# paulvoliva/XNODE-WAN-PDE-solver

Measured on AMD Instinct MI355X. Metric: WAN training-steps/sec (optimiser sub-steps, d=20 cube, N_r=4096 paths per GPU), higher is better.
Workload: dtype f64

## Files before the change

### include/xnwan.h

```cpp
#ifndef XNWAN_H
#define XNWAN_H
#ifdef __cplusplus
extern "C" {
#endif

#define XW_E_DIMS     (-1)
#define XW_E_ARG      (-2)
#define XW_E_WORKSPACE (-3)
#define XW_E_COMM     (-4)

int xw_abi_version(void);
int xw_supported_dims(char* buf, int buflen);

int xw_theta_size(int d, int H, int K);
int xw_phi_size(int d, int W);

int xw_ode_fwd(const double* xT, const double* t, const double* start, const double* theta,
               int method, int N, int L, int d, int H, int K, int m,
               double* u, double* Y, void* stream);

typedef struct { const double* xT; const double* start; double* u; double* Y; double* act; int N;
                 int act_x_only;
                 int narrow;
                 int prio_drop;
               } XwOdeFwdJob;
int xw_ode_act_rows(int method, int H, int K, int m);
int xw_ode_fwd_multi(const XwOdeFwdJob* jobs, int njobs, const double* t, const double* theta,
                     int method, int L, int d, int H, int K, int m, double* zero16, void* stream);

int xw_ode_bwd_slabs(int N);

int xw_ode_bwd(const double* xT, const double* t, const double* start, const double* theta, const double* Y,
               const double* ubar, int method, int N, int L, int d, int H, int K, int m, int mode,
               double* gx, double* gs, double* gslab, void* stream);

typedef struct { const double* xT; const double* start; const double* Y; const double* act; const double* ubar;
                 double* gx; double* gs; double* gslab; int N;
                 int res_first_only; const double* res_u; const double* res_ref; double res_coef; double res_base;
                 int res_w_per_point; const double* res_w; const double* res_c; const double* res_cp; double res_kappa2;
               } XwOdeBwdJob;
int xw_ode_bwd_multi(const XwOdeBwdJob* jobs, int njobs, const double* t, const double* theta,
                     int method, int L, int d, int H, int K, int m, int mode, void* stream);

int xw_tiled_ode_ok(int d, int H, int K, int m);
int xw_tiled_ode_work(int sweep, int d, int H, int K, int m);
int xw_tiled_ode_bwd_slabs(int N);
int xw_tiled_ode_fwd_multi(const XwOdeFwdJob* jobs, int njobs, const double* t, const double* theta,
                           int method, int L, int d, int H, int K, int m, double* zero16, double* work, void* stream);
int xw_tiled_ode_bwd_multi(const XwOdeBwdJob* jobs, int njobs, const double* t, const double* theta,
                           int method, int L, int d, int H, int K, int m, int mode, double* work, void* stream);

int xw_adams_coef(int k, double* out);
int xw_adams_tiled_work(int sweep, int d, int H, int K, int m);
int xw_adams_tiled_fwd_multi(const XwOdeFwdJob* jobs, int njobs, const double* t, const double* theta,
                             int L, int d, int H, int K, int m, double* zero16, double* work, void* stream);
int xw_adams_tiled_bwd_multi(const XwOdeBwdJob* jobs, int njobs, const double* t, const double* theta,
                             int L, int d, int H, int K, int m, int mode, double* work, void* stream);

#define XW_DOPRI_CTL 16
#define XW_DOPRI_UNDERFLOW 1
#define XW_DOPRI_STEPS 2
#define XW_DOPRI_NONFINITE 3
#define XW_DOPRI_CAPACITY 4
typedef struct { const double* xT; const double* start; double* u; double* Y; double* rec_y; double* rec_t; double* rec_h;
                 double* fbuf; double* ctl; double* work; int N; int cap; } XwDopriJob;
int xw_dopri5_ctl_size(void);
int xw_dopri5_work_size(int N);
int xw_dopri5_init(const XwDopriJob* jobs, int njobs, const double* t, const double* theta, int L, int d, int H, int K, int m,
                   int Hn, double rtol, double atol, void* stream);
int xw_dopri5_attempts(const XwDopriJob* jobs, int njobs, const double* t, const double* theta, int L, int d, int H, int K,
                       int m, int Hn, double rtol, double atol, int max_steps, int n, void* stream);
typedef struct { XwOdeBwdJob b; const double* rec_y; const double* rec_t; const double* rec_h; const double* ctl; } XwDopriSweepJob;
int xw_dopri5_sweep(const XwDopriSweepJob* jobs, int njobs, const double* t, const double* theta, int L, int d, int H, int K,
                    int m, int mode, void* stream);

int xw_tdopri5_work(int sweep, int d, int H, int K, int m);
int xw_tdopri5_part_size(int N);
int xw_tdopri5_init(const XwDopriJob* jobs, int njobs, const double* t, const double* theta, int L, int d, int H, int K, int m,
                    int Hn, double rtol, double atol, double* work, void* stream);
int xw_tdopri5_attempts(const XwDopriJob* jobs, int njobs, const double* t, const double* theta, int L, int d, int H, int K,
                        int m, int Hn, double rtol, double atol, int max_steps, int n, double* work, void* stream);
int xw_tdopri5_sweep(const XwDopriSweepJob* jobs, int njobs, const double* t, const double* theta, int L, int d, int H, int K,
                     int m, int mode, double* work, void* stream);

int xw_disc_fwd(const double* xT, const double* t, const double* tpp, const double* phi,
                int N, int L, int d, int W, int q, double* v, double* vt, double* gxv, double* gtv, int ngrad,
                int max_blocks, double* act, void* stream);
int xw_disc_xproj(const double* xT, const double* phi, int N, int d, int W, double* xproj, void* stream);
int xw_disc_fwd_xproj(const double* xT, const double* t, const double* tpp, const double* phi,
                      int N, int L, int d, int W, int q, double* v, double* vt, double* gxv, double* gtv, int ngrad,
                      int max_blocks, double* act, const double* xproj, void* stream);
int xw_disc_act_rows(int W, int q);

int xw_disc_gradx(const double* xT, const double* t, const double* tpp, const double* phi, const double* vbar,
                  int N, int d, int W, int q, double* gxv, double* gtv, void* stream);

int xw_disc_bwd_slabs(int N, int L);
int xw_disc_bwd(const double* xT, const double* t, const double* tpp, const double* phi, const double* vbar,
                int N, int L, int d, int W, int q, const double* act, double* gslab, void* stream);

int xw_disc_tiled_ok(int d, int W, int q);
int xw_disc_tiled_act_rows(int W, int q);
int xw_disc_tiled_fwd(const double* xT, const double* t, const double* tpp, const double* phi,
                      int N, int L, int d, int W, int q, double* v, double* vt, double* gxv, double* gtv, int ngrad,
                      int max_blocks, double* act, const double* xproj, void* stream);
int xw_disc_tiled_bwd(const double* xT, const double* t, const double* tpp, const double* phi, const double* vbar,
                      int N, int L, int d, int W, int q, const double* act, double* gslab, void* stream);

int xw_weak_partials(const double* u, const double* v, const double* vt, const double* w, int w_per_point,
                     const double* wt, const double* s3x, const double* gx, const double* gs, const double* ghT,
                     const double* gxv, const double* w0, const double* gwx0T, int d, const double* c, double ckappa,
                     const double* f, const double* h, const double* href, int pairwise, double s3_scale, int N, int L,
                     double Vol, double Nglob, double* work, double* scal, int finalize, int Lb, double Nbglob, double alpha,
                     double init_off, double bdry_off, long long* step, const double* ub, const double* gb, long Pb,
                     void* stream);
int xw_pair_fold(double* scal, double Vol, double Nglob, void* stream);
int xw_reduce_work_size(void);
int xw_cube_weight(const float* x, int N, int d, double top, double bot, double* w, double* w0, double* gwT, double* xT,
                   void* stream);
int xw_weak_contract_general(const double* A0, int amode, const double* B0, const double* gx, const double* gs,
                             const double* ghT, const double* gxv, const double* w0, const double* gwx0T, const double* v0,
                             int d, int N, double* s3x, void* stream);
int xw_bdry_partials(const double* ub, const double* g, int Nb, int L, double alpha, double Nbglob,
                     double* ubar_b, double* work, double* scal, void* stream);
int xw_gen_cotangents(const double* u, const double* v, const double* w, int w_per_point, const double* c,
                      const double* cp, double ckappa, const double* h, int N, int L, double Vol, double Nglob,
                      double alpha, double pollution, const double* scal, double* ubarA, double* ubarB, void* stream);
int xw_disc_cotangent(const double* u, const double* v, const double* w, int w_per_point, const double* c,
                      double ckappa, const double* f, const double* h, int N, int L, double Vol, double Nglob,
                      double pollution, double s3_scale, const double* scal_in, double* vbar, void* stream);
int xw_losses(double* scal, int L, int Lb, double Vol, double Nglob, double Nbglob, double alpha, double init_off,
              double bdry_off, long long* step, void* stream);

int xw_adam(double* param, const double* gslabA, int nA, const double* gextraA, const double* gslabB, int nB,
            const double* gextraB, const double* scal, double* m, double* v, long long* step, int bump_step, int P,
            double lr, double beta1, double beta2, double eps, double* gsum_out, int lag_lo, int lag_hi, int skip,
            long long* lag, void* stream);
int xw_slab_sum(const double* gslab, int nslab, int P, int accumulate, double* out, void* stream);
int xw_slab_sum2(const double* gA, int nA, double* outA, const double* gB, int nB, double* outB, int P, void* stream);

typedef struct {
  int N, Nb, L, Lb, d;
  int same_grid;
  int w_per_point, amode, pair_i, pair_b;
  int ns_u, ns_b;
  int narrow;
  int sharded;
  double Vol, Nglob, Nbglob, s3_scale, init_off, bdry_off, ckappa;
  const double *xT, *xvT, *xbT, *t, *tb, *tpp, *xvT_pts;
  const double *start, *start_b, *h, *href, *f, *g, *w, *wt, *w0, *ghT, *gwx0T, *c, *cp, *A0, *B0;
  double *u, *ub, *Y, *Yb, *act, *act_b, *v, *vt, *gxv, *gtv, *gx, *gs, *vbar, *s3x, *vact, *slabA, *slabB, *slab_v, *work_i, *work_b;
  double *xproj;
} XwGroup;
typedef int (*XwExchangeFn)(double* buf, int count, void* ctx, void* stream);
typedef struct {
  int method, H, K, m, W, q, Pu, Pv, adjoint;
  int v_blocks, v_blocks_disc;
  int lag_lo, lag_hi;
  double alpha, pollution, lr_u, lr_v, beta1, beta2, eps;
  double *theta, *phi, *scal, *grad_u, *grad_v, *m_u, *v_u, *m_v, *v_v;
  long long *step_u, *step_v, *lag_u;
  XwExchangeFn exchange;
  void* exchange_ctx;
  double* pack_u;
} XwSolverState;
int xw_substep_gen(const XwGroup* g, const XwSolverState* s, int skip_v, int store_record, double* accum, int adam_skip_field,
                   void* stream);
int xw_substep_disc(const XwGroup* g, const XwSolverState* s, int skip_v, int use_record, double* accum, void* stream);

int xw_comm_available(void);
int xw_comm_unique_id(unsigned char* id128);
int xw_comm_init(const unsigned char* id128, int nranks, int rank, void** comm);
int xw_allreduce(double* buf, int count, void* comm, void* stream);
int xw_comm_destroy(void* comm);

typedef struct XwGather {
  const double* src;
  double* dst;
  long n0, n1, n2;
  long s0, s1, s2;
  long before;
} XwGather;
int xw_gather_fields(const XwGather* table_dev, int count, long total, void* stream);

int xw_mt19937_uniform_f32(void* state_blob, long blob_bytes, float* out, long n, float from, float to, int fused);

int xw_mt19937_legacy_normal_f64(unsigned int* key, int* pos, int* has_gauss, double* cached_gaussian, double* out, long n);

#ifdef __cplusplus
}
#endif
#endif
```

### xnode_wan_pde_solver_amd/_lib.py

```python
import ctypes
import os

_HERE = os.path.dirname(os.path.abspath(__file__))
LIB_PATH = os.environ.get('XW_LIBRARY') or os.path.join(_HERE, 'libxnwan.so')
ABI_VERSION = 33

c_f32p = ctypes.c_void_p
c_f64p = ctypes.c_void_p
c_i64p = ctypes.c_void_p
c_int, c_dbl, c_vp = ctypes.c_int, ctypes.c_double, ctypes.c_void_p


class XwOdeFwdJob(ctypes.Structure):
    _fields_ = [('xT', c_vp), ('start', c_vp), ('u', c_vp), ('Y', c_vp), ('act', c_vp), ('N', c_int), ('act_x_only', c_int),
                ('narrow', c_int), ('prio_drop', c_int)]


class XwOdeBwdJob(ctypes.Structure):
    _fields_ = [('xT', c_vp), ('start', c_vp), ('Y', c_vp), ('act', c_vp), ('ubar', c_vp), ('gx', c_vp), ('gs', c_vp),
                ('gslab', c_vp), ('N', c_int), ('res_first_only', c_int), ('res_u', c_vp), ('res_ref', c_vp),
                ('res_coef', ctypes.c_double), ('res_base', ctypes.c_double), ('res_w_per_point', c_int), ('res_w', c_vp),
                ('res_c', c_vp), ('res_cp', c_vp), ('res_kappa2', ctypes.c_double)]


class XwDopriJob(ctypes.Structure):
    _fields_ = [('xT', c_vp), ('start', c_vp), ('u', c_vp), ('Y', c_vp), ('rec_y', c_vp), ('rec_t', c_vp), ('rec_h', c_vp),
                ('fbuf', c_vp), ('ctl', c_vp), ('work', c_vp), ('N', c_int), ('cap', c_int)]


class XwDopriSweepJob(ctypes.Structure):
    _fields_ = [('b', XwOdeBwdJob), ('rec_y', c_vp), ('rec_t', c_vp), ('rec_h', c_vp), ('ctl', c_vp)]


class XwGroup(ctypes.Structure):
    _fields_ = ([(n, c_int) for n in ('N', 'Nb', 'L', 'Lb', 'd', 'same_grid', 'w_per_point', 'amode', 'pair_i', 'pair_b', 'ns_u', 'ns_b',
                                      'narrow', 'sharded')]
                + [(n, c_dbl) for n in ('Vol', 'Nglob', 'Nbglob', 's3_scale', 'init_off', 'bdry_off', 'ckappa')]
                + [(n, c_vp) for n in ('xT', 'xvT', 'xbT', 't', 'tb', 'tpp', 'xvT_pts', 'start', 'start_b', 'h', 'href', 'f', 'g', 'w',
                                       'wt', 'w0', 'ghT', 'gwx0T', 'c', 'cp', 'A0', 'B0', 'u', 'ub', 'Y', 'Yb', 'act', 'act_b', 'v',
                                       'vt', 'gxv', 'gtv', 'gx', 'gs', 'vbar', 's3x', 'vact', 'slabA', 'slabB', 'slab_v', 'work_i',
                                       'work_b', 'xproj')])


class XwSolverState(ctypes.Structure):
    _fields_ = ([(n, c_int) for n in ('method', 'H', 'K', 'm', 'W', 'q', 'Pu', 'Pv', 'adjoint', 'v_blocks', 'v_blocks_disc', 'lag_lo',
                                      'lag_hi')]
                + [(n, c_dbl) for n in ('alpha', 'pollution', 'lr_u', 'lr_v', 'beta1', 'beta2', 'eps')]
                + [(n, c_vp) for n in ('theta', 'phi', 'scal', 'grad_u', 'grad_v', 'm_u', 'v_u', 'm_v', 'v_v', 'step_u', 'step_v',
                                       'lag_u', 'exchange', 'exchange_ctx', 'pack_u')])


EXCHANGE_FN = ctypes.CFUNCTYPE(ctypes.c_int, ctypes.c_void_p, ctypes.c_int, ctypes.c_void_p, ctypes.c_void_p)


SIGNATURES = {
    'xw_abi_version': [],
    'xw_supported_dims': [ctypes.c_char_p, c_int],
    'xw_theta_size': [c_int, c_int, c_int],
    'xw_phi_size': [c_int, c_int],
    'xw_ode_fwd': [c_f32p, c_f32p, c_f64p, c_f64p, c_int, c_int, c_int, c_int, c_int, c_int, c_int, c_f64p, c_f64p, c_vp],
    'xw_ode_fwd_multi': [ctypes.POINTER(XwOdeFwdJob), c_int, c_f32p, c_f64p, c_int, c_int, c_int, c_int, c_int, c_int, c_f64p,
                         c_vp],
    'xw_ode_bwd_slabs': [c_int],
    'xw_ode_act_rows': [c_int, c_int, c_int, c_int],
    'xw_ode_bwd_multi': [ctypes.POINTER(XwOdeBwdJob), c_int, c_f32p, c_f64p, c_int, c_int, c_int, c_int, c_int, c_int, c_int, c_vp],
    'xw_tiled_ode_ok': [c_int, c_int, c_int, c_int],
    'xw_tiled_ode_work': [c_int, c_int, c_int, c_int, c_int],
    'xw_tiled_ode_bwd_slabs': [c_int],
    'xw_tiled_ode_fwd_multi': [ctypes.POINTER(XwOdeFwdJob), c_int, c_f32p, c_f64p, c_int, c_int, c_int, c_int, c_int, c_int, c_f64p,
                               c_f64p, c_vp],
    'xw_tiled_ode_bwd_multi': [ctypes.POINTER(XwOdeBwdJob), c_int, c_f32p, c_f64p, c_int, c_int, c_int, c_int, c_int, c_int, c_int,
                               c_f64p, c_vp],
    'xw_adams_coef': [c_int, c_vp],
    'xw_adams_tiled_work': [c_int, c_int, c_int, c_int, c_int],
    'xw_adams_tiled_fwd_multi': [ctypes.POINTER(XwOdeFwdJob), c_int, c_f32p, c_f64p, c_int, c_int, c_int, c_int, c_int, c_f64p, c_f64p,
                                 c_vp],
    'xw_adams_tiled_bwd_multi': [ctypes.POINTER(XwOdeBwdJob), c_int, c_f32p, c_f64p, c_int, c_int, c_int, c_int, c_int, c_int, c_f64p,
                                 c_vp],
    'xw_dopri5_ctl_size': [],
    'xw_dopri5_work_size': [c_int],
    'xw_dopri5_init': [ctypes.POINTER(XwDopriJob), c_int, c_f32p, c_f64p, c_int, c_int, c_int, c_int, c_int, c_int, c_dbl, c_dbl,
                       c_vp],
    'xw_dopri5_attempts': [ctypes.POINTER(XwDopriJob), c_int, c_f32p, c_f64p, c_int, c_int, c_int, c_int, c_int, c_int, c_dbl,
                           c_dbl, c_int, c_int, c_vp],
    'xw_dopri5_sweep': [ctypes.POINTER(XwDopriSweepJob), c_int, c_f32p, c_f64p, c_int, c_int, c_int, c_int, c_int, c_int, c_vp],
    'xw_tdopri5_work': [c_int, c_int, c_int, c_int, c_int],
    'xw_tdopri5_part_size': [c_int],
    'xw_tdopri5_init': [ctypes.POINTER(XwDopriJob), c_int, c_f32p, c_f64p, c_int, c_int, c_int, c_int, c_int, c_int, c_dbl, c_dbl,
                        c_f64p, c_vp],
    'xw_tdopri5_attempts': [ctypes.POINTER(XwDopriJob), c_int, c_f32p, c_f64p, c_int, c_int, c_int, c_int, c_int, c_int, c_dbl,
                            c_dbl, c_int, c_int, c_f64p, c_vp],
    'xw_tdopri5_sweep': [ctypes.POINTER(XwDopriSweepJob), c_int, c_f32p, c_f64p, c_int, c_int, c_int, c_int, c_int, c_int, c_f64p,
                         c_vp],
    'xw_ode_bwd': [c_f32p, c_f32p, c_f64p, c_f64p, c_f64p, c_f64p, c_int, c_int, c_int, c_int, c_int, c_int, c_int, c_int,
                   c_f64p, c_f64p, c_f64p, c_vp],
    'xw_disc_fwd': [c_f32p, c_f32p, c_f32p, c_f64p, c_int, c_int, c_int, c_int, c_int, c_f64p, c_f64p, c_f64p, c_f64p, c_int,
                    c_int, c_f64p, c_vp],
    'xw_disc_xproj': [c_f32p, c_f64p, c_int, c_int, c_int, c_f64p, c_vp],
    'xw_disc_fwd_xproj': [c_f32p, c_f32p, c_f32p, c_f64p, c_int, c_int, c_int, c_int, c_int, c_f64p, c_f64p, c_f64p, c_f64p, c_int,
                          c_int, c_f64p, c_f64p, c_vp],
    'xw_disc_act_rows': [c_int, c_int],
    'xw_disc_gradx': [c_f32p, c_f32p, c_f32p, c_f64p, c_f64p, c_int, c_int, c_int, c_int, c_f64p, c_f64p, c_vp],
    'xw_disc_bwd_slabs': [c_int, c_int],
    'xw_disc_bwd': [c_f32p, c_f32p, c_f32p, c_f64p, c_f64p, c_int, c_int, c_int, c_int, c_int, c_f64p, c_f64p, c_vp],
    'xw_disc_tiled_ok': [c_int, c_int, c_int],
    'xw_disc_tiled_act_rows': [c_int, c_int],
    'xw_disc_tiled_fwd': [c_f32p, c_f32p, c_f32p, c_f64p, c_int, c_int, c_int, c_int, c_int, c_f64p, c_f64p, c_f64p, c_f64p, c_int,
                          c_int, c_f64p, c_f64p, c_vp],
    'xw_disc_tiled_bwd': [c_f32p, c_f32p, c_f32p, c_f64p, c_f64p, c_int, c_int, c_int, c_int, c_int, c_f64p, c_f64p, c_vp],
    'xw_mt19937_uniform_f32': [c_vp, ctypes.c_long, c_vp, ctypes.c_long, ctypes.c_float, ctypes.c_float, c_int],
    'xw_gather_fields': [c_vp, c_int, ctypes.c_long, c_vp],
    'xw_mt19937_legacy_normal_f64': [c_vp, ctypes.POINTER(c_int), ctypes.POINTER(c_int), ctypes.POINTER(c_dbl), c_vp, ctypes.c_long],
    'xw_weak_partials': [c_f64p, c_f64p, c_f64p, c_f64p, c_int, c_f64p, c_f64p, c_f64p, c_f64p, c_f64p, c_f64p, c_f64p,
                         c_f64p, c_int, c_f64p, c_dbl, c_f64p, c_f64p, c_f64p, c_int, c_dbl, c_int, c_int, c_dbl, c_dbl, c_f64p, c_f64p,
                         c_int, c_int, c_dbl, c_dbl, c_dbl, c_dbl, c_i64p, c_f64p, c_f64p, ctypes.c_long, c_vp],
    'xw_pair_fold': [c_f64p, c_dbl, c_dbl, c_vp],
    'xw_cube_weight': [c_vp, c_int, c_int, c_dbl, c_dbl, c_f64p, c_f64p, c_f64p, c_f64p, c_vp],
    'xw_bdry_partials': [c_f64p, c_f64p, c_int, c_int, c_dbl, c_dbl, c_f64p, c_f64p, c_f64p, c_vp],
    'xw_reduce_work_size': [],
    'xw_weak_contract_general': [c_f64p, c_int, c_f64p, c_f64p, c_f64p, c_f64p, c_f64p, c_f64p, c_f64p, c_f64p, c_int, c_int, c_f64p, c_vp],
    'xw_gen_cotangents': [c_f64p, c_f64p, c_f64p, c_int, c_f64p, c_f64p, c_dbl, c_f64p, c_int, c_int, c_dbl, c_dbl, c_dbl,
                          c_dbl, c_f64p, c_f64p, c_f64p, c_vp],
    'xw_disc_cotangent': [c_f64p, c_f64p, c_f64p, c_int, c_f64p, c_dbl, c_f64p, c_f64p, c_int, c_int, c_dbl, c_dbl, c_dbl,
                          c_dbl, c_f64p, c_f64p, c_vp],
    'xw_losses': [c_f64p, c_int, c_int, c_dbl, c_dbl, c_dbl, c_dbl, c_dbl, c_dbl, c_i64p, c_vp],
    'xw_adam': [c_f64p, c_f64p, c_int, c_f64p, c_f64p, c_int, c_f64p, c_f64p, c_f64p, c_f64p, c_i64p, c_int, c_int, c_dbl,
                c_dbl, c_dbl, c_dbl, c_f64p, c_int, c_int, c_int, c_i64p, c_vp],
    'xw_substep_gen': [ctypes.POINTER(XwGroup), ctypes.POINTER(XwSolverState), c_int, c_int, c_f64p, c_int, c_vp],
    'xw_substep_disc': [ctypes.POINTER(XwGroup), ctypes.POINTER(XwSolverState), c_int, c_int, c_f64p, c_vp],
    'xw_slab_sum': [c_f64p, c_int, c_int, c_int, c_f64p, c_vp],
    'xw_slab_sum2': [c_f64p, c_int, c_f64p, c_f64p, c_int, c_f64p, c_int, c_vp],
    'xw_comm_available': [],
# ... 45 lines not shown
```

### xnode_wan_pde_solver_amd/csrc/xw_common.h

```cpp
#pragma once
#include <hip/hip_runtime.h>

typedef double d4 __attribute__((ext_vector_type(4)));
#define XW_MFMA(a, b, c) __builtin_amdgcn_mfma_f64_16x16x4f64((a), (b), (c), 0, 0, 0)
#define XW_MFMA4(a, b, c) __builtin_amdgcn_mfma_f64_4x4x4f64((a), (b), (c), 0, 0, 0)

#define XW_E_DIMS (-1)
#define XW_ODE_MAX_LAYERS 10
#define XW_E_ARG (-2)
#define XW_E_WORKSPACE (-3)
#define XW_E_COMM (-4)

struct UOff {
  int IL0w, IL0b, IL2w, IL2b, IL4w, IL4b, Win, Winb, Wh, Whb, Wo, Wob, FLw, FLb, total, ldin;
};
__host__ __device__ inline UOff u_offsets(int d, int H, int K) {
  UOff o;
  int p = 0;
  o.IL0w = p; p += H;
  o.IL0b = p; p += H;
  o.IL2w = p; p += H * H;
  o.IL2b = p; p += H;
  o.IL4w = p; p += H * H;
  o.IL4b = p; p += H;
  o.ldin = d + 1 + H;
  o.Win = p; p += K * o.ldin;
  o.Winb = p; p += K;
  o.Wh = p; p += K * K;
  o.Whb = p; p += K;
  o.Wo = p; p += H * K;
  o.Wob = p; p += H;
  o.FLw = p; p += H;
  o.FLb = p; p += 1;
  o.total = p;
  return o;
}
struct VOff {
  int Vin, Vinb, Vh, Vhb, Vo, Vob, total, ldin;
};
__host__ __device__ inline VOff v_offsets(int d, int W) {
  VOff o;
  int p = 0;
  o.ldin = d + 1;
  o.Vin = p; p += W * o.ldin;
  o.Vinb = p; p += W;
  o.Vh = p; p += W * W;
  o.Vhb = p; p += W;
  o.Vo = p; p += W;
  o.Vob = p; p += 1;
  o.total = p;
  return o;
}

typedef const double __attribute__((address_space(1)))* xw_gcp;
typedef double __attribute__((address_space(1)))* xw_gp;
__device__ __forceinline__ double xw_ld_g(const double* p) { return *(xw_gcp)p; }
__device__ __forceinline__ void xw_st_g(double v, double* p) { *(xw_gp)p = v; }
__device__ __forceinline__ double xw_ld_nt(const double* p) { return __builtin_nontemporal_load((xw_gcp)p); }
__device__ __forceinline__ void xw_st_nt(double v, double* p) { __builtin_nontemporal_store(v, (xw_gp)p); }

__device__ __forceinline__ int xw_lane() { return threadIdx.x & 63; }

__device__ __forceinline__ double xw_fragA(const double* __restrict__ Mx, int ld, int rows, int cols, int r0, int c0) {
  const int l = xw_lane();
  const int r = r0 + (l & 15), c = c0 + (l >> 4);
  return (r < rows && c < cols) ? xw_ld_g(Mx + (r * ld + c)) : 0.0;
}
__device__ __forceinline__ double xw_fragAT(const double* __restrict__ Mx, int ld, int rows, int cols, int r0, int c0) {
  const int l = xw_lane();
  const int r = r0 + (l & 15), c = c0 + (l >> 4);
  return (r < cols && c < rows) ? xw_ld_g(Mx + (c * ld + r)) : 0.0;
}
__device__ __forceinline__ double xw_fragAT_l(const double* __restrict__ Mx, int ld, int rows, int cols, int r0, int c0, int l) {
  const int r = r0 + (l & 15), c = c0 + (l >> 4);
  return (r < cols && c < rows) ? xw_ld_g(Mx + (c * ld + r)) : 0.0;
}
__device__ __forceinline__ double xw_fragA4(const double* __restrict__ Mx, int ld, int rows, int cols, int r0, int c0) {
  const int l = xw_lane();
  const int r = r0 + (l & 3), c = c0 + (l >> 4);
  return (r < rows && c < cols) ? xw_ld_g(Mx + (r * ld + c)) : 0.0;
}
__device__ __forceinline__ double xw_fragAT4(const double* __restrict__ Mx, int ld, int rows, int cols, int r0, int c0) {
  const int l = xw_lane();
  const int r = r0 + (l & 3), c = c0 + (l >> 4);
  return (r < cols && c < rows) ? xw_ld_g(Mx + (c * ld + r)) : 0.0;
}
__device__ __forceinline__ double xw_relu1(double x) { return __builtin_fmax(x, 0.0); }
__device__ __forceinline__ d4 xw_vecD(const double* __restrict__ b, int rows, int r0) {
  const int g = xw_lane() >> 4;
  d4 v;
#pragma unroll
  for (int r = 0; r < 4; ++r) {
    const int i = r0 + g + 4 * r;
    v[r] = (i < rows) ? xw_ld_g(b + i) : 0.0;
  }
  return v;
}
__device__ __forceinline__ d4 xw_vecD_strided(const double* __restrict__ b, int stride, int rows, int r0) {
  const int g = xw_lane() >> 4;
  d4 v;
#pragma unroll
  for (int r = 0; r < 4; ++r) {
    const int i = r0 + g + 4 * r;
    v[r] = (i < rows) ? xw_ld_g(b + (long)i * stride) : 0.0;
  }
  return v;
}
__device__ __forceinline__ d4 xw_relu(d4 z) {
  d4 o;
#pragma unroll
  for (int r = 0; r < 4; ++r) o[r] = z[r] > 0.0 ? z[r] : 0.0;
  return o;
}
__device__ __forceinline__ double xw_gate_pos(double b, double x) {
  const unsigned t = (unsigned)__double2loint(b) | (unsigned)__double2hiint(b);
  const int m = -(int)(t < 1u ? t : 1u);
  return __hiloint2double(__double2hiint(x) & m, __double2loint(x) & m);
}
__device__ __forceinline__ d4 xw_zero4() { d4 z = {0.0, 0.0, 0.0, 0.0}; return z; }

__device__ __forceinline__ double xw_tanh(double x) {
  const double am = fmin(fabs(x), 40.0);
  const double y = -2.0 * am;
  const double nb = fma(y, 1.4426950408889634, 6755399441055744.0);
  const double n = nb - 6755399441055744.0;
  double r = fma(n, -6.93147180369123816490e-01, y);
  r = fma(n, -1.90821492927058770002e-10, r);
  double p = 2.08767569878681e-09;
  p = fma(p, r, 2.505210838544172e-08);
  p = fma(p, r, 2.755731922398589e-07);
  p = fma(p, r, 2.7557319223985893e-06);
  p = fma(p, r, 2.48015873015873e-05);
  p = fma(p, r, 0.0001984126984126984);
  p = fma(p, r, 0.001388888888888889);
  p = fma(p, r, 0.008333333333333333);
  p = fma(p, r, 0.041666666666666664);
  p = fma(p, r, 0.16666666666666666);
  p = fma(p, r, 0.5);
  p = fma(p, r, 1.0);
  p = fma(p, r, 1.0);
  const double e = __hiloint2double(__double2hiint(p) + (__double2loint(nb) << 20), __double2loint(p));
  const double num = 1.0 - e, den = 1.0 + e;
// ... 74 lines not shown
```

### xnode_wan_pde_solver_amd/csrc/xw_dopri.hip

```cpp
#include "xw_common.h"
#include "xnwan.h"
#include "xw_generic.h"

namespace {
#include "xw_generic_field.h"
#include "xw_generic_cot.h"

#include "xw_dopri_ctl.h"

__device__ __forceinline__ void put_output(const XwDopriJob& j, const double* flw, double flb, int l, int H, int path,
                                           const double* y) {
  double acc = flb;
  for (int h = 0; h < H; ++h) acc = fma(flw[h], y[h], acc);
  j.u[(long)l * j.N + path] = acc;
  if (j.Y)
    for (int h = 0; h < H; ++h) j.Y[((long)l * H + h) * j.N + path] = y[h];
}

template <int HM>
__global__ void __launch_bounds__(64) kd_init1(const Jobs<XwDopriJob> J, const double* __restrict__ tf, const double* __restrict__ theta,
                                               int L, int d, int H, int K, int m, int Hn, double rtol, double atol) {
  int lb;
  const XwDopriJob& j = J.j[job_of(J, lb)];
  const int N = j.N, nb = (N + 63) / 64, raw = lb * 64 + (int)threadIdx.x;
// ... 302 lines not shown
  const double* Win = theta + n.o.Win;
  if (slab) {
    gadd_run(slab, n.o.Winb, K, active, [&](int q) { return Sx[q]; });
    for (int q = 0; q < K; ++q) {
      const double sq = Sx[q];
      gadd_run(slab, n.o.Win + q * n.o.ldin, d, active, [&](int i) { return sq * job.xT[(long)i * N + path]; });
    }
  }
  if (want_x && job.gx != nullptr && active)
    for (int i = 0; i < d; ++i) {
      double acc = 0.0;
      for (int q = 0; q < K; ++q) acc = fma(Win[q * n.o.ldin + i], Sx[q], acc);
      job.gx[(long)i * N + path] = acc;
    }
}

bool dims_ok(int L, int d, int H, int K, int m, int Hn) { return L >= 1 && xwg_ode_ok(d, H, K, m) && Hn >= 1 && Hn <= H; }

int fwd_jobs(const XwDopriJob* jobs, int njobs, Jobs<XwDopriJob>& P) {
  int e = pack_jobs(jobs, njobs, P);
  if (e) return e;
  for (int i = 0; i < njobs; ++i) {
    const XwDopriJob& j = jobs[i];
    if (!j.xT || !j.start || !j.u || !j.rec_y || !j.rec_t || !j.rec_h || !j.fbuf || !j.ctl || !j.work || j.N < 1 || j.cap < 0)
      return XW_E_ARG;
    P.blk0[i + 1] = P.blk0[i] + (j.N + 63) / 64;
  }
  return 0;
}
}

extern "C" int xw_dopri5_ctl_size(void) { return XW_DOPRI_CTL; }
extern "C" int xw_dopri5_work_size(int N) { return N < 1 ? XW_E_ARG : 2 * ((N + 63) / 64); }

extern "C" int xw_dopri5_init(const XwDopriJob* jobs, int njobs, const double* t, const double* theta, int L, int d, int H, int K,
                              int m, int Hn, double rtol, double atol, void* stream) {
  if (!t || !theta || !(rtol >= 0.0) || !(atol >= 0.0)) return XW_E_ARG;
  if (!dims_ok(L, d, H, K, m, Hn)) return XW_E_DIMS;
  Jobs<XwDopriJob> P;
  const int e = fwd_jobs(jobs, njobs, P);
  if (e) return e;
  hipStream_t s = (hipStream_t)stream;
  const dim3 g(P.blk0[njobs]), b(64);
  if (H <= 32) {
    hipLaunchKernelGGL(kd_init1<32>, g, b, 0, s, P, t, theta, L, d, H, K, m, Hn, rtol, atol);
    hipLaunchKernelGGL(kd_init2<32>, g, b, 0, s, P, t, theta, L, d, H, K, m, Hn, rtol, atol);
  } else {
    hipLaunchKernelGGL(kd_init1<64>, g, b, 0, s, P, t, theta, L, d, H, K, m, Hn, rtol, atol);
    hipLaunchKernelGGL(kd_init2<64>, g, b, 0, s, P, t, theta, L, d, H, K, m, Hn, rtol, atol);
  }
  return xw_launch_status();
}

extern "C" int xw_dopri5_attempts(const XwDopriJob* jobs, int njobs, const double* t, const double* theta, int L, int d, int H,
                                  int K, int m, int Hn, double rtol, double atol, int max_steps, int n, void* stream) {
  if (!t || !theta || !(rtol >= 0.0) || !(atol >= 0.0) || max_steps < 1 || n < 0) return XW_E_ARG;
  if (!dims_ok(L, d, H, K, m, Hn)) return XW_E_DIMS;
  Jobs<XwDopriJob> P;
  const int e = fwd_jobs(jobs, njobs, P);
  if (e) return e;
  hipStream_t s = (hipStream_t)stream;
  const dim3 g(P.blk0[njobs]), b(64);
  for (int i = 0; i < n; ++i) {
    if (H <= 32)
      hipLaunchKernelGGL(kd_attempt<32>, g, b, 0, s, P, t, theta, L, d, H, K, m, Hn, rtol, atol, max_steps);
    else
      hipLaunchKernelGGL(kd_attempt<64>, g, b, 0, s, P, t, theta, L, d, H, K, m, Hn, rtol, atol, max_steps);
  }
  return xw_launch_status();
}

extern "C" int xw_dopri5_sweep(const XwDopriSweepJob* jobs, int njobs, const double* t, const double* theta, int L, int d, int H,
                               int K, int m, int mode, void* stream) {
  if (!t || !theta || L < 1 || (mode & ~7) || ((mode & 4) && (mode & 3) != 3)) return XW_E_ARG;
  if (!xwg_ode_ok(d, H, K, m)) return XW_E_DIMS;
  Jobs<XwDopriSweepJob> P;
  int e = pack_jobs(jobs, njobs, P);
  if (e) return e;
  hipStream_t s = (hipStream_t)stream;
  const long Pu = u_offsets(d, H, K).total;
  for (int i = 0; i < njobs; ++i) {
    const XwDopriSweepJob& j = jobs[i];
    if (!j.b.xT || !j.b.start || !j.rec_y || !j.rec_t || !j.rec_h || !j.ctl || j.b.N < 1) return XW_E_ARG;
    if (j.b.res_u != nullptr && j.b.ubar != nullptr) return XW_E_ARG;
    if ((mode & 2) && !j.b.gslab) return XW_E_ARG;
    if ((mode & 1) && !(mode & 4) && (!j.b.gx || !j.b.gs)) return XW_E_ARG;
    if (mode & 2) {
      const hipError_t he = hipMemsetAsync(j.b.gslab, 0, sizeof(double) * Pu * ((j.b.N + 15) / 16), s);
      if (he != hipSuccess) return (int)he;
    }
    P.blk0[i + 1] = P.blk0[i] + (j.b.N + 63) / 64;
  }
  const dim3 g(P.blk0[njobs]), b(64);
  if (H <= 32)
    hipLaunchKernelGGL(kd_sweep<32>, g, b, 0, s, P, t, theta, L, d, H, K, m, mode);
  else
    hipLaunchKernelGGL(kd_sweep<64>, g, b, 0, s, P, t, theta, L, d, H, K, m, mode);
  return xw_launch_status();
}
```

### xnode_wan_pde_solver_amd/csrc/xw_generic.hip

```cpp
#include "xw_common.h"
#include "xnwan.h"
#include "xw_generic.h"

namespace {
#include "xw_generic_field.h"

__device__ void rk_step(const Net& n, int method, const double* xproj, double t0, double dt, double* y) {
  const int H = n.H;
  double k1[GH], k2[GH], k3[GH], tmp[GH];
  field_eval(n, xproj, t0, y, k1, nullptr);
  if (method == 0) {
    for (int j = 0; j < H; ++j) y[j] = fma(dt, k1[j], y[j]);
  } else if (method == 1) {
    for (int j = 0; j < H; ++j) tmp[j] = fma(k1[j], dt / 2, y[j]);
    field_eval(n, xproj, t0 + dt / 2, tmp, k2, nullptr);
    for (int j = 0; j < H; ++j) y[j] = fma(dt, k2[j], y[j]);
  } else {
    for (int j = 0; j < H; ++j) tmp[j] = y[j] + dt * k1[j] / 3;
    field_eval(n, xproj, t0 + dt / 3, tmp, k2, nullptr);
    for (int j = 0; j < H; ++j) tmp[j] = y[j] + dt * (k2[j] - k1[j] / 3);
    field_eval(n, xproj, t0 + 2 * dt / 3, tmp, k3, nullptr);
    for (int j = 0; j < H; ++j) tmp[j] = y[j] + dt * (k1[j] - k2[j] + k3[j]);
    double k4[GH];
    field_eval(n, xproj, t0 + dt, tmp, k4, nullptr);
// ... 294 lines not shown
        dj[kk] = r[(long)kk * cols] > 0.0 ? a0 : 0.0;
        if (kk + 1 < W) dj[kk + 1] = r[(long)(kk + 1) * cols] > 0.0 ? a1 : 0.0;
        if (kk + 2 < W) dj[kk + 2] = r[(long)(kk + 2) * cols] > 0.0 ? a2 : 0.0;
        if (kk + 3 < W) dj[kk + 3] = r[(long)(kk + 3) * cols] > 0.0 ? a3 : 0.0;
      }
    }
    for (int k = 0; k < W; k += 4) {
      double dk[4][GQ];
#pragma unroll
      for (int j = 0; j < GQ; ++j)
#pragma unroll
        for (int i = 0; i < 4; ++i) dk[i][j] = (j < q && k + i < W) ? dls[(j + 1) * GW + k + i] : 0.0;
      const int lane = threadIdx.x;
      for (int c = 0; c < W; c += 64) {
        double mine[4] = {0.0, 0.0, 0.0, 0.0};
        for (int i = 0; i < 64; ++i) {
          if (c + i >= W) break;
          double a0 = 0.0, a1 = 0.0, a2 = 0.0, a3 = 0.0;
#pragma unroll
          for (int j = 0; j < GQ; ++j) {
            if (j < q) {
              const double rj = act[((long)j * W + c + i) * cols + p];
              a0 = fma(dk[0][j], rj, a0);
              a1 = fma(dk[1][j], rj, a1);
              a2 = fma(dk[2][j], rj, a2);
              a3 = fma(dk[3][j], rj, a3);
            }
          }
          a0 = gsum64(a0); a1 = gsum64(a1); a2 = gsum64(a2); a3 = gsum64(a3);
          if (lane == i) { mine[0] = a0; mine[1] = a1; mine[2] = a2; mine[3] = a3; }
        }
        if (c + lane < W) {
#pragma unroll
          for (int i = 0; i < 4; ++i)
            if (k + i < W) slab[o.Vh + (k + i) * W + c + lane] += mine[i];
        }
      }
    }
    wadd_run(slab, o.Vhb, W, [&](int k) {
      double acc = 0.0;
      for (int j = 0; j < q; ++j) acc += dls[(j + 1) * GW + k];
      return acc;
    });
    wadd_run(slab, o.Vinb, W, [&](int k) { return dls[k]; });
    for (int k = 0; k < W; ++k) {
      const double d0 = dls[k];
      wadd_run(slab, o.Vin + k * o.ldin, 1 + d, [&](int c) { return d0 * (c == 0 ? t : xT[(long)(c - 1) * N + nidx]); });
    }
  }
}

}

int xwg_ode_ok(int d, int H, int K, int m) { return H >= 1 && H <= GH && K >= 1 && K <= GK && m >= 1 && m <= GM && d >= 1 && d + 2 <= 128; }
int xwg_disc_ok(int d, int W, int q) { return W >= 1 && W <= GW && q >= 0 && q <= GQ && d >= 1 && d + 2 <= 128; }

int xwg_ode_fwd_multi(const XwOdeFwdJob* jobs, int njobs, const double* t, const double* theta, int method, int L, int d, int H,
                      int K, int m, double* zero16, void* stream) {
  if (!jobs || njobs < 1 || !t || !theta || L < 1 || method < 0 || method > 2) return XW_E_ARG;
  if (!xwg_ode_ok(d, H, K, m)) return XW_E_DIMS;
  hipStream_t s = (hipStream_t)stream;
  if (zero16 != nullptr) {
    const hipError_t e = hipMemsetAsync(zero16, 0, 16 * sizeof(double), s);
    if (e != hipSuccess) return (int)e;
  }
  for (int i = 0; i < njobs; ++i) {
    const XwOdeFwdJob& j = jobs[i];
    if (!j.xT || !j.start || !j.u || j.N < 1) return XW_E_ARG;
    hipLaunchKernelGGL(kg_ode_fwd, dim3((j.N + 63) / 64), dim3(64), 0, s, j, t, theta, method, L, d, H, K, m);
  }
  return xw_launch_status();
}

int xwg_ode_bwd_multi(const XwOdeBwdJob* jobs, int njobs, const double* t, const double* theta, int method, int L, int d, int H,
                      int K, int m, int mode, void* stream) {
  if (!jobs || njobs < 1 || !t || !theta || L < 1 || method < 0 || method > 2 || (mode & 3) == 0) return XW_E_ARG;
  if (!xwg_ode_ok(d, H, K, m) || (mode & 8)) return XW_E_DIMS;
  if ((mode & 4) && (mode & 3) != 3) return XW_E_ARG;
  hipStream_t s = (hipStream_t)stream;
  const long P = u_offsets(d, H, K).total;
  for (int i = 0; i < njobs; ++i) {
    const XwOdeBwdJob& j = jobs[i];
    if (!j.xT || !j.start || !j.Y || j.N < 1) return XW_E_ARG;
    if (j.res_u != nullptr && j.ubar != nullptr) return XW_E_ARG;
    if ((mode & 2) && !j.gslab) return XW_E_ARG;
    if ((mode & 1) && !(mode & 4) && (!j.gx || !j.gs)) return XW_E_ARG;
    if (mode & 2) {
      const hipError_t e = hipMemsetAsync(j.gslab, 0, sizeof(double) * P * ((j.N + 15) / 16), s);
      if (e != hipSuccess) return (int)e;
    }
    hipLaunchKernelGGL(kg_ode_bwd, dim3((j.N + 63) / 64), dim3(64), 0, s, j, t, theta, method, L, d, H, K, m, mode);
  }
  return xw_launch_status();
}

int xwg_disc_fwd(const double* xT, const double* t, const double* tpp, const double* phi, int N, int L, int d, int W, int q,
                 double* v, double* vt, double* gxv, double* gtv, int ngrad, double* act, void* stream) {
  if (!xwg_disc_ok(d, W, q)) return XW_E_DIMS;
  const long P = (long)N * L;
  const long cols = (P + 15) / 16 * 16;
  hipLaunchKernelGGL(kg_disc_fwd, dim3((unsigned)((P + 63) / 64)), dim3(64), 0, (hipStream_t)stream, xT, t, tpp, phi, N, L, d, W, q, v,
                     vt, gxv, gtv, ngrad, act, cols);
  return xw_launch_status();
}

int xwg_disc_bwd(const double* xT, const double* t, const double* tpp, const double* phi, const double* vbar, int N, int L, int d,
                 int W, int q, const double* act, double* gslab, int nslab, void* stream) {
  if (!xwg_disc_ok(d, W, q)) return XW_E_DIMS;
  if (!act) return XW_E_DIMS;
  const long P = (long)N * L;
  const long cols = (P + 15) / 16 * 16;
  const hipError_t e = hipMemsetAsync(gslab, 0, sizeof(double) * (size_t)v_offsets(d, W).total * nslab, (hipStream_t)stream);
  if (e != hipSuccess) return (int)e;
  hipLaunchKernelGGL(kg_disc_bwd, dim3(nslab), dim3(64), 0, (hipStream_t)stream, xT, t, tpp, phi, vbar, N, L, d, W, q, act, cols, gslab);
  return xw_launch_status();
}
```

### xnode_wan_pde_solver_amd/csrc/xw_generic_cot.h

```cpp
#pragma once
__device__ double cot_u(const XwOdeBwdJob& j, int l, int L, int path) {
  const long p = (long)l * j.N + path;
  if (j.res_u == nullptr) return j.ubar ? j.ubar[p] : 1.0;
  if (j.res_first_only == 2) {
    const double u = j.res_u[p], v = j.res_ref[p];
    const double w = j.res_w_per_point ? j.res_w[p] : j.res_w[path];
    const double dcu = j.res_c != nullptr ? j.res_c[p] + u * j.res_cp[p] : j.res_kappa2 * u;
    double g = j.res_coef * dcu * v * w;
    if (l == L - 1) g += j.res_base * v;
    return g;
  }
  if (j.res_first_only == 1) return l == 0 ? j.res_base + j.res_coef * (j.res_u[p] - j.res_ref[path]) : j.res_base;
  return j.res_base + j.res_coef * (j.res_u[p] - j.res_ref[p]);
}
```

### xnode_wan_pde_solver_amd/csrc/xw_ode.hip

```cpp
#include <cstdlib>
#include <type_traits>
#include "xw_common.h"
#ifndef XW_ODE_FWD_WAVES
#define XW_ODE_FWD_WAVES 2
#endif
#include "xnwan.h"

#if !defined(XW_ODE_H) || !defined(XW_ODE_K)
#error "compile with -DXW_ODE_H=<u_hidden_dim> -DXW_ODE_K=<u_hidden_hidden_dim>"
#endif
#ifdef XW_ODE_WIDE16
#define XW_ODE_FORM "xw_ode_mfma16.h"
#else
#define XW_ODE_FORM "xw_ode_mfma4.h"
#endif
#define XW_CAT4_(a, b, c, d) a##b##c##d
#define XW_CAT4(a, b, c, d) XW_CAT4_(a, b, c, d)
#define XW_ODE_FN(name) XW_CAT4(name, XW_ODE_H, _, XW_ODE_K)
#ifdef XW_ODE_ONLY_M
#define XW_ODE_DISPATCH(CALL)                                    \
  switch (m) {                                                   \
    case XW_ODE_ONLY_M: { CALL(XW_ODE_H, XW_ODE_K, XW_ODE_ONLY_M) } \
    default: return XW_E_DIMS;                                   \
  }
// ... 179 lines not shown
#pragma unroll
  for (int ks = 0; ks < 4; ++ks) acc = XW_MFMA(a[ks], b[ks], acc);
  __builtin_amdgcn_sched_barrier(0);
}
#define XW_SWEEP_TILES 6

#define XW_ODE_SECTION 1
#include XW_ODE_FORM
template <int H, int K>
__device__ __forceinline__ void lift(const double* __restrict__ th, const UOff& o, double sv, d4 (&a0)[Dim<H, K>::HT],
                                     d4 (&a1)[Dim<H, K>::HT], d4 (&y)[Dim<H, K>::HT]) {
  typedef Dim<H, K> D;
#pragma unroll
  for (int ht = 0; ht < D::HT; ++ht)
    a0[ht] = xw_relu(xw_vecD(th + o.IL0w, H, 16 * ht) * sv + xw_vecD(th + o.IL0b, H, 16 * ht));
#pragma unroll
  for (int ht = 0; ht < D::HT; ++ht) {
    d4 v = xw_vecD(th + o.IL2b, H, 16 * ht);
#pragma unroll
    for (int ks = 0; ks < D::KSH; ++ks) v = XW_MFMA(xw_fragA(th + o.IL2w, H, H, H, 16 * ht, 4 * ks), a0[ks >> 2][ks & 3], v);
    a1[ht] = xw_relu(v);
  }
#pragma unroll
  for (int ht = 0; ht < D::HT; ++ht) {
    d4 v = xw_vecD(th + o.IL4b, H, 16 * ht);
#pragma unroll
    for (int ks = 0; ks < D::KSH; ++ks) v = XW_MFMA(xw_fragA(th + o.IL4w, H, H, H, 16 * ht, 4 * ks), a1[ks >> 2][ks & 3], v);
    y[ht] = v;
  }
}

template <int H, int K>
__device__ __forceinline__ d4 project_x(const double* __restrict__ th, const UOff& o, const double* __restrict__ xT,
                                        int N, int d, int ncl) {
  const int g = xw_lane() >> 4;
  d4 xp = xw_vecD(th + o.Winb, K, 0);
  for (int ks = 0; ks < (d + 3) / 4; ++ks) {
    const int i = 4 * ks + g;
    const double b = i < d ? xT[(long)i * N + ncl] : 0.0;
    xp = XW_MFMA(xw_fragA(th + o.Win, o.ldin, K, d, 0, 4 * ks), b, xp);
  }
  return xp;
}

#define XW_MAXJOBS 4
struct FwdJobs {
  const double* xT[XW_MAXJOBS];
  const double* start[XW_MAXJOBS];
  double* u[XW_MAXJOBS];
  double* Y[XW_MAXJOBS];
  double* act[XW_MAXJOBS];
  int N[XW_MAXJOBS];
  int tile0[XW_MAXJOBS + 1];
  int n;
  int x_only;
  int narrow;
  int prio;
  double* zero16;
};
struct BwdJobs {
  const double* xT[XW_MAXJOBS];
  const double* start[XW_MAXJOBS];
  const double* Y[XW_MAXJOBS];
  const double* act[XW_MAXJOBS];
  const double* ubar[XW_MAXJOBS];
  double* gx[XW_MAXJOBS];
  double* gs[XW_MAXJOBS];
  double* gslab[XW_MAXJOBS];
  int N[XW_MAXJOBS];
  int tile0[XW_MAXJOBS + 1];
  int n;
  int x_ones;
  int prio;
  int spread;
  const double* res_u[XW_MAXJOBS];
  const double* res_ref[XW_MAXJOBS];
  double res_coef[XW_MAXJOBS], res_base[XW_MAXJOBS];
  int res_first[XW_MAXJOBS];
  const double* res_w[XW_MAXJOBS];
  const double* res_c[XW_MAXJOBS];
  const double* res_cp[XW_MAXJOBS];
  double res_kappa2[XW_MAXJOBS];
  int res_wpp[XW_MAXJOBS];
};
__device__ __forceinline__ double cot_u(const BwdJobs& jobs, int job, const double* __restrict__ ubar, int l, int N, int col,
                                        int L) {
  const double* __restrict__ ru = jobs.res_u[job];
  if (ru != nullptr) {
    if (jobs.res_first[job] == 2) {
      const long p = (long)l * N + col;
      const double ul = ru[p], vl = jobs.res_ref[job][p];
      const double wl = jobs.res_wpp[job] ? jobs.res_w[job][p] : jobs.res_w[job][col];
      const double dcu = jobs.res_c[job] != nullptr ? jobs.res_c[job][p] + ul * jobs.res_cp[job][p] : jobs.res_kappa2[job] * ul;
      double gB = jobs.res_coef[job] * dcu * vl * wl;
      if (l == L - 1) gB += jobs.res_base[job] * vl;
      return gB;
    }
    double r = jobs.res_base[job];
    if (jobs.res_first[job]) {
      if (l == 0) r += jobs.res_coef[job] * (ru[col] - jobs.res_ref[job][col]);
    } else {
      r += jobs.res_coef[job] * (ru[(long)l * N + col] - jobs.res_ref[job][(long)l * N + col]);
    }
    return r;
  }
  return ubar != nullptr ? ubar[(long)l * N + col] : 1.0;
}
struct Cot4 {
  const double *p0, *p1, *p2, *p3, *p4;
  long s0, s1, s2;
  double cb, coef, base, kappa2;
  bool weak, use_st, use_res, first, tab, valid;
};
struct CotRaw { double a, b, c, d, e; };
__device__ __forceinline__ Cot4 make_cot(const BwdJobs& jobs, int job, int N, int col, bool valid, const double* dummy) {
  Cot4 c;
  const double* ru = jobs.res_u[job];
  const double* ubar = jobs.ubar[job];
  c.valid = valid;
  c.weak = ru != nullptr && jobs.res_first[job] == 2;
  c.use_res = ru != nullptr && !c.weak;
  c.use_st = ru == nullptr && ubar != nullptr;
  c.first = c.use_res && jobs.res_first[job] != 0;
  c.cb = ru != nullptr ? jobs.res_base[job] : (ubar != nullptr ? 0.0 : 1.0);
  c.coef = jobs.res_coef[job];
  c.base = jobs.res_base[job];
  c.kappa2 = jobs.res_kappa2[job];
  c.tab = c.weak && jobs.res_c[job] != nullptr;
  if (c.weak) {
    c.p0 = ru + col; c.p1 = jobs.res_ref[job] + col; c.p2 = jobs.res_w[job] + col;
    c.p3 = (c.tab ? jobs.res_c[job] : ru) + col; c.p4 = (c.tab ? jobs.res_cp[job] : ru) + col;
    c.s0 = N; c.s1 = N; c.s2 = jobs.res_wpp[job] ? N : 0;
  } else {
    c.p0 = (c.use_st ? ubar : dummy) + col; c.s0 = c.use_st ? N : 0;
    c.p1 = (c.use_res ? ru : dummy) + col; c.p2 = (c.use_res ? jobs.res_ref[job] : dummy) + col;
    c.s1 = (c.use_res && !c.first) ? N : 0; c.s2 = 0;
    c.p3 = c.p4 = dummy;
  }
  return c;
}
template <bool WEAK> __device__ __forceinline__ CotRaw cot_issue(const Cot4& c, int l) {
  CotRaw r;
  r.a = xw_ld_g(c.p0 + l * c.s0);
  r.b = xw_ld_g(c.p1 + l * c.s1);
  if (WEAK) {
    r.c = xw_ld_g(c.p2 + l * c.s2);
    r.d = xw_ld_g(c.p3 + l * c.s1);
    r.e = xw_ld_g(c.p4 + l * c.s1);
  } else {
    r.c = xw_ld_g(c.p2 + l * c.s1);
    r.d = r.e = 0.0;
  }
  return r;
}
template <bool WEAK> __device__ __forceinline__ double cot_value(const Cot4& c, const CotRaw& r, int l, int L) {
  double ub;
  if (WEAK) {
    const double dcu = c.tab ? fma(r.a, r.e, r.d) : c.kappa2 * r.a;
    ub = c.coef * dcu * r.b * r.c;
    if (l == L - 1) ub = fma(c.base, r.b, ub);
  } else {
    ub = c.cb;
    if (c.use_st) ub += r.a;
    if (c.use_res && (!c.first || l == 0)) ub = fma(c.coef, r.b - r.c, ub);
  }
  return c.valid ? ub : 0.0;
}

template <typename J> __device__ __forceinline__ int find_job(const J& jobs, int vb) {
  int j = 0;
#pragma unroll
  for (int k = 1; k < XW_MAXJOBS; ++k)
    if (k < jobs.n && vb >= jobs.tile0[k]) j = k;
  return j;
}

#define XW_ODE_PRIO 3
__device__ __forceinline__ void xw_setprio(int p) {
  if (p >= 3) __builtin_amdgcn_s_setprio(3);
  else if (p == 2) __builtin_amdgcn_s_setprio(2);
  else if (p == 1) __builtin_amdgcn_s_setprio(1);
}

template <int H, int K, int M, int S> struct ActLayout {
  static constexpr int STAGE = M * K;
  static constexpr int YI = S * STAGE;
  static constexpr int ROWS = S * STAGE + (S - 1) * H;
  static constexpr int MASK = ROWS;
  static constexpr int MR = 2 * XW_MASK_WORDS(M);
  static constexpr int TOTAL = ROWS + MR * S;
};
struct ActLane {
  unsigned off;
  unsigned off_part;
  unsigned off_part_st;
  bool valid;
};
#define XW_ACT_OOB 0x7fffff00u
__device__ __forceinline__ ActLane act_lane(int N, int col, bool valid, int krows) {
  const int g = xw_lane() >> 4, p = krows & 3;
  const int gp = p ? (g < p ? g : p - 1) : g;
  const unsigned part = 8u * (unsigned)((p ? p : 4) * col + gp);
  return ActLane{8u * (unsigned)(4 * col + g), part, (p == 0 || g < p) ? part : XW_ACT_OOB, valid};
}
typedef unsigned xw_u2v __attribute__((ext_vector_type(2)));
struct ActBuf {
  __amdgpu_buffer_rsrc_t rsrc;
};
__device__ __forceinline__ ActBuf act_buf(double* A, int bytes) {
  return ActBuf{__builtin_amdgcn_make_buffer_rsrc(A, 0, bytes, 0x00020000)};
}
__device__ __forceinline__ void act_store(const ActBuf& B, int row0, int nrows, int N, const ActLane& q, d4 v) {
#pragma unroll
  for (int r = 0; r < 4; ++r)
    if (4 * r < nrows) {
      const int so = (row0 + 4 * r) * N * 8;
      const double x = v[r];
      const xw_u2v w2 = {(unsigned)__double2loint(x), (unsigned)__double2hiint(x)};
      __builtin_amdgcn_raw_buffer_store_b64(w2, B.rsrc, (int)(4 * r + 4 <= nrows ? q.off : q.off_part_st), so, 2);
    }
}
__device__ __forceinline__ d4 act_load(const double* __restrict__ A, int row0, int nrows, int N, const ActLane& q) {
  d4 v = xw_zero4();
  const char* base = reinterpret_cast<const char*>(A + (long)row0 * N);
#pragma unroll
  for (int r = 0; r < 4; ++r)
    if (4 * r < nrows) {
      const char* __restrict__ blk = base + (long)(4 * r) * N * 8;
      v[r] = __builtin_nontemporal_load(reinterpret_cast<const double*>(blk + (4 * r + 4 <= nrows ? q.off : q.off_part)));
    }
  return v;
}

template <int K, int M, bool FULL = true> struct SinkAct {
  const ActBuf& A;
  int row0, N;
  const ActLane& q;
  unsigned& bits;
  unsigned& bits_hi;
  __device__ __forceinline__ double relu(int, int kb, double z) const {
    const bool kb_last = kb == (K + 3) / 4 - 1;
    const unsigned long long open = __builtin_amdgcn_ballot_w64(z > 0.0);
    double r;
    if constexpr (XW_MASK_WORDS(M) == 2) {
      if (kb_last) asm("v_addc_co_u32_e64 %1, vcc, %1, %1, %4\n\tv_addc_co_u32_e64 %2, vcc, %2, %2, vcc\n\tv_max_f64 %0, %3, 0\n\ts_nop 1" : "=v"(r), "+v"(bits), "+v"(bits_hi) : "v"(z), "s"(open) : "vcc");
      else asm("v_addc_co_u32_e64 %1, vcc, %1, %1, %4\n\tv_addc_co_u32_e64 %2, vcc, %2, %2, vcc\n\tv_max_f64 %0, %3, 0" : "=v"(r), "+v"(bits), "+v"(bits_hi) : "v"(z), "s"(open) : "vcc");
      return r;
// ... 682 lines not shown
  for (int i = 0; i < jobs.n; ++i) act = act && jobs.act[i] != nullptr;
  const int sel = method * 3 + (act ? (jobs.x_only ? 2 : 1) : 0);
  int rc;
  if (launch_fwd_narrow<H, K, M>(sel, jobs, t, theta, L, d, grid, s, rc)) return rc;
  switch (sel) {
    case 0: hipLaunchKernelGGL((k_ode_fwd<H, K, M, 0, 0>), grid, block, 0, s, jobs, t, theta, L, d); break;
    case 1: hipLaunchKernelGGL((k_ode_fwd<H, K, M, 0, 1>), grid, block, 0, s, jobs, t, theta, L, d); break;
    case 2: hipLaunchKernelGGL((k_ode_fwd<H, K, M, 0, 2>), grid, block, 0, s, jobs, t, theta, L, d); break;
    case 3: hipLaunchKernelGGL((k_ode_fwd<H, K, M, 1, 0>), grid, block, 0, s, jobs, t, theta, L, d); break;
    case 4: hipLaunchKernelGGL((k_ode_fwd<H, K, M, 1, 1>), grid, block, 0, s, jobs, t, theta, L, d); break;
    case 5: hipLaunchKernelGGL((k_ode_fwd<H, K, M, 1, 2>), grid, block, 0, s, jobs, t, theta, L, d); break;
    case 6: hipLaunchKernelGGL((k_ode_fwd<H, K, M, 2, 0>), grid, block, 0, s, jobs, t, theta, L, d); break;
    default: return XW_E_ARG;
  }
  return xw_launch_status();
}

}

#ifndef XW_ODE_PART_RECOMP
extern "C" int XW_ODE_FN(xw_ode_fwd_multi_w)(const XwOdeFwdJob* jobs, int njobs, const double* t, const double* theta, int method,
                                             int L, int d, int m, double* zero16, void* stream) {
  if (!jobs || njobs < 1 || njobs > XW_MAXJOBS || !t || !theta || L <= 0 || d <= 0 || m < 1) return XW_E_ARG;
  FwdJobs J;
  J.n = njobs;
  J.zero16 = zero16;
  J.x_only = jobs[0].act_x_only ? 1 : 0;
  J.narrow = jobs[0].narrow ? 1 : 0;
  J.prio = XW_ODE_PRIO - (jobs[0].prio_drop < 0 ? 0 : jobs[0].prio_drop > 3 ? 3 : jobs[0].prio_drop);
  J.tile0[0] = 0;
  for (int i = 0; i < XW_MAXJOBS; ++i) {
    const bool on = i < njobs;
    if (on && (!jobs[i].xT || !jobs[i].start || !jobs[i].u || jobs[i].N <= 0)) return XW_E_ARG;
    if (on && (jobs[i].act_x_only ? 1 : 0) != J.x_only) return XW_E_ARG;
    if (on && (jobs[i].narrow ? 1 : 0) != J.narrow) return XW_E_ARG;
    J.xT[i] = on ? jobs[i].xT : nullptr;
    J.start[i] = on ? jobs[i].start : nullptr;
    J.u[i] = on ? jobs[i].u : nullptr;
    J.Y[i] = on ? jobs[i].Y : nullptr;
    J.act[i] = (on && method != 2) ? jobs[i].act : nullptr;
    if (on && (J.act[i] != nullptr) != (J.act[0] != nullptr)) return XW_E_ARG;
    J.N[i] = on ? jobs[i].N : 0;
    J.tile0[i + 1] = J.tile0[i] + (on ? (jobs[i].N + 15) / 16 : 0);
  }
  hipStream_t s = (hipStream_t)stream;
#define CALL(HH, KK, MM) return launch_fwd<HH, KK, MM>(method, J, t, theta, L, d, s);
  XW_ODE_DISPATCH(CALL)
#undef CALL
}

extern "C" int XW_ODE_FN(xw_ode_bwd_multi_w)(const XwOdeBwdJob* jobs, int njobs, const double* t, const double* theta, int method,
                                             int L, int d, int m, int mode, void* stream) {
  if (!jobs || njobs < 1 || njobs > XW_MAXJOBS || !t || !theta || L <= 0 || d <= 0 || m < 1 || (mode & 3) == 0 || ((mode & 4) && (mode & 3) != 3) || ((mode & 8) && (mode & 4)) || ((mode & 16) && (mode & 8)) || (mode & ~127)) return XW_E_ARG;
  BwdJobs J;
  J.n = njobs;
  J.x_ones = (mode & 4) ? 1 : 0;
  J.spread = 0;
  J.prio = XW_ODE_PRIO - ((mode >> 5) & 3);
  J.tile0[0] = 0;
  for (int i = 0; i < XW_MAXJOBS; ++i) {
    const bool on = i < njobs;
    if (on) {
      if (!jobs[i].xT || !jobs[i].start || !jobs[i].Y || jobs[i].N <= 0) return XW_E_ARG;
      if ((mode & 2) && !jobs[i].gslab) return XW_E_ARG;
      if ((mode & 1) && !(mode & 4) && (!jobs[i].gx || !jobs[i].gs)) return XW_E_ARG;
      if ((mode & 1) && (!jobs[i].gx != !jobs[i].gs)) return XW_E_ARG;
    }
    J.xT[i] = on ? jobs[i].xT : nullptr;
    J.start[i] = on ? jobs[i].start : nullptr;
    J.Y[i] = on ? jobs[i].Y : nullptr;
    J.act[i] = (on && method != 2 && !(mode & 8)) ? jobs[i].act : nullptr;
    if (on && (J.act[i] != nullptr) != (J.act[0] != nullptr)) return XW_E_ARG;
    J.ubar[i] = on ? jobs[i].ubar : nullptr;
    J.res_u[i] = on ? jobs[i].res_u : nullptr;
    J.res_ref[i] = on ? jobs[i].res_ref : nullptr;
    J.res_coef[i] = on ? jobs[i].res_coef : 0.0;
    J.res_base[i] = on ? jobs[i].res_base : 0.0;
    J.res_first[i] = on ? jobs[i].res_first_only : 0;
    J.res_w[i] = on ? jobs[i].res_w : nullptr;
    J.res_c[i] = on ? jobs[i].res_c : nullptr;
    J.res_cp[i] = on ? jobs[i].res_cp : nullptr;
    J.res_kappa2[i] = on ? jobs[i].res_kappa2 : 0.0;
    J.res_wpp[i] = on ? jobs[i].res_w_per_point : 0;
    if (on && jobs[i].res_u && (!jobs[i].res_ref || jobs[i].ubar)) return XW_E_ARG;
    if (on && jobs[i].res_u && jobs[i].res_first_only == 2 && (!jobs[i].res_w || (!jobs[i].res_c != !jobs[i].res_cp))) return XW_E_ARG;
    if (on && (jobs[i].res_first_only < 0 || jobs[i].res_first_only > 2)) return XW_E_ARG;
    J.gx[i] = (on && (mode & 1)) ? jobs[i].gx : nullptr;
    J.gs[i] = (on && (mode & 1)) ? jobs[i].gs : nullptr;
    J.gslab[i] = (on && (mode & 2)) ? jobs[i].gslab : nullptr;
    J.N[i] = on ? jobs[i].N : 0;
    J.tile0[i + 1] = J.tile0[i] + (on ? (jobs[i].N + 15) / 16 : 0);
  }
  hipStream_t s = (hipStream_t)stream;
#define CALL(HH, KK, MM)                                                             \
  return (mode & 2) ? launch_bwd<HH, KK, MM, true>(method, J, t, theta, L, d, (mode & 8) != 0, (mode & 16) != 0, s)     \
                    : launch_bwd<HH, KK, MM, false>(method, J, t, theta, L, d, (mode & 8) != 0, (mode & 16) != 0, s);
  XW_ODE_DISPATCH(CALL)
#undef CALL
}
#else
extern "C" int XW_ODE_FN(xw_ode_bwd_recomp_w)(const void* jobs_, const double* t, const double* theta, int method, int L, int d,
                                              int m, int params, int adj, void* stream) {
  const BwdJobs& jobs = *static_cast<const BwdJobs*>(jobs_);
  const dim3 grid(jobs.tile0[jobs.n]), block(64);
  hipStream_t s = (hipStream_t)stream;
#define LAUNCH(HH, KK, MM, PP, AA)                                                                                                 \
  switch (method) {                                                                                                                \
    case 0: hipLaunchKernelGGL((k_ode_bwd<HH, KK, MM, 0, PP, false, AA>), grid, block, 0, s, jobs, t, theta, L, d); break;         \
    case 1: hipLaunchKernelGGL((k_ode_bwd<HH, KK, MM, 1, PP, false, AA>), grid, block, 0, s, jobs, t, theta, L, d); break;         \
    case 2: hipLaunchKernelGGL((k_ode_bwd<HH, KK, MM, 2, PP, false, AA>), grid, block, 0, s, jobs, t, theta, L, d); break;         \
    default: return XW_E_ARG;                                                                                                      \
  }                                                                                                                                \
  return xw_launch_status();
#define CALL(HH, KK, MM)                                                                                                           \
  if (params && adj) { LAUNCH(HH, KK, MM, true, true) }                                                                            \
  else if (params) { LAUNCH(HH, KK, MM, true, false) }                                                                             \
  else if (adj) { LAUNCH(HH, KK, MM, false, true) }                                                                                \
  else { LAUNCH(HH, KK, MM, false, false) }
  XW_ODE_DISPATCH(CALL)
#undef CALL
#undef LAUNCH
}
#endif
```

### xnode_wan_pde_solver_amd/csrc/xw_substep.hip

```cpp
#include <hip/hip_runtime.h>
#include <string.h>
#include "xnwan.h"

namespace {
struct Side {
  hipStream_t s = nullptr;
  hipEvent_t fork = nullptr, fwd = nullptr, done = nullptr;
};
Side* side_of_current_device() {
  static Side sides[64];
  int dev = 0;
  if (hipGetDevice(&dev) != hipSuccess || dev < 0 || dev >= 64) return nullptr;
  Side& x = sides[dev];
  if (x.s == nullptr) {
    if (hipStreamCreateWithFlags(&x.s, hipStreamNonBlocking) != hipSuccess) return nullptr;
    if (hipEventCreateWithFlags(&x.fork, hipEventDisableTiming) != hipSuccess || hipEventCreateWithFlags(&x.fwd, hipEventDisableTiming) != hipSuccess ||
        hipEventCreateWithFlags(&x.done, hipEventDisableTiming) != hipSuccess)
      return nullptr;
  }
  return &x;
}
#define XW_HIP(call) { const hipError_t e_ = (call); if (e_ != hipSuccess) return (int)e_; }

inline XwOdeFwdJob fwd_job(const double* xT, const double* start, double* u, double* Y, double* act, int N, int x_only, int narrow) {
  XwOdeFwdJob j;
  j.xT = xT; j.start = start; j.u = u; j.Y = Y; j.act = act; j.N = N; j.act_x_only = x_only; j.narrow = narrow; j.prio_drop = 0;
  return j;
}
inline XwOdeBwdJob bwd_job(const double* xT, const double* start, const double* Y, const double* act, int N) {
  XwOdeBwdJob j;
  memset(&j, 0, sizeof(j));
  j.xT = xT; j.start = start; j.Y = Y; j.act = act; j.N = N;
  return j;
}
#define XW_TRY(call) { const int rc_ = (call); if (rc_ != 0) return rc_; }

int test_net(const XwGroup* g, const XwSolverState* s, int blocks, double* record, void* stream) {
  if (g->tpp != nullptr)
    return xw_disc_fwd(g->xvT_pts, nullptr, g->tpp, s->phi, g->N * g->L, 1, g->d, s->W, s->q, g->v, g->vt, g->gxv, g->gtv, g->N, blocks,
                       record, stream);
  if (g->xproj != nullptr) XW_TRY(xw_disc_xproj(g->xvT, s->phi, g->N, g->d, s->W, g->xproj, stream));
  return xw_disc_fwd_xproj(g->xvT, g->t, nullptr, s->phi, g->N, g->L, g->d, s->W, s->q, g->v, g->vt, g->gxv, g->gtv, g->N, blocks, record,
                           g->xproj, stream);
}
int contract(const XwGroup* g, const XwSolverState* s, long long* step, bool with_bdry, bool finalize, void* stream) {
  const double* s3x = nullptr;
  if (g->A0 != nullptr || g->B0 != nullptr) {
    XW_TRY(xw_weak_contract_general(g->A0, g->amode, g->B0, g->gx, g->gs, g->ghT, g->gxv, g->w0, g->gwx0T, g->v, g->d, g->N, g->s3x,
                                    stream));
    s3x = g->s3x;
  }
  const bool fused = s3x == nullptr;
  return xw_weak_partials(g->u, g->v, g->vt, g->w, g->w_per_point, g->wt, s3x, fused ? g->gx : nullptr, fused ? g->gs : nullptr,
                          fused ? g->ghT : nullptr, fused ? g->gxv : nullptr, fused ? g->w0 : nullptr, fused ? g->gwx0T : nullptr,
                          fused ? g->d : 0, g->c, g->ckappa, g->f, g->h, g->pair_i ? g->href : nullptr, g->pair_i ? 1 : 0,
                          g->pair_i ? g->s3_scale : 1.0, g->N, g->L, g->Vol, g->Nglob, g->work_i, s->scal, finalize ? 1 : 0,
                          g->Lb > 0 ? g->Lb : 1, g->Nbglob, s->alpha, g->init_off, g->bdry_off, finalize ? step : nullptr, with_bdry && g->Nb > 0 ? g->ub : nullptr,
                          with_bdry && g->Nb > 0 ? g->g : nullptr, with_bdry && g->Nb > 0 ? (long)g->Nb * g->Lb : 0, stream);
}
inline bool sharded(const XwGroup* g, const XwSolverState* s) { return g->sharded != 0 && s->exchange != nullptr; }
#define XW_ZERO(ptr, count) XW_HIP(hipMemsetAsync((ptr), 0, sizeof(double) * (size_t)(count), (hipStream_t)stream))
}

extern "C" int xw_substep_gen(const XwGroup* g, const XwSolverState* s, int skip_v, int store_record, double* accum,
                              int adam_skip_field, void* stream) {
  if (!g || !s || g->N < 0 || g->Nb < 0 || g->L <= 0) return XW_E_ARG;
  const bool shard = sharded(g, s);
  if (g->N == 0 && !shard) return XW_E_ARG;
  if (shard && (!s->pack_u || s->scal != s->pack_u + 2 * (long)s->Pu)) return XW_E_ARG;
  const bool fused_x = s->pollution == 1.0 && !s->adjoint;
  const bool have_i = g->N > 0, have_b = g->Nb > 0;
  const bool joint = have_i && have_b && g->same_grid;
  const int adj = s->adjoint ? 8 : 0;
  void* const main_stream = stream;
  if (have_i) {
    Side* sd = side_of_current_device();
    if (sd == nullptr) return XW_E_ARG;
    XW_HIP(hipEventRecord(sd->fork, (hipStream_t)main_stream));
    XW_HIP(hipStreamWaitEvent(sd->s, sd->fork, 0));
    if (!skip_v) XW_TRY(test_net(g, s, s->v_blocks, store_record ? g->vact : nullptr, main_stream));
    stream = (void*)sd->s;
    {
      XwOdeFwdJob jobs[2] = {fwd_job(g->xT, g->start, g->u, g->Y, g->act, g->N, 0, (g->narrow >> 0) & 1),
                             fwd_job(g->xbT, g->start_b, g->ub, g->Yb, g->act_b, g->Nb, 0, (g->narrow >> 0) & 1)};
      XW_TRY(xw_ode_fwd_multi(jobs, joint ? 2 : 1, g->t, s->theta, s->method, g->L, g->d, s->H, s->K, s->m, s->scal, stream));
      if (have_b && !joint) {
        XwOdeFwdJob jb = fwd_job(g->xbT, g->start_b, g->ub, g->Yb, g->act_b, g->Nb, 0, (g->narrow >> 1) & 1);
        XW_TRY(xw_ode_fwd_multi(&jb, 1, g->tb, s->theta, s->method, g->Lb, g->d, s->H, s->K, s->m, nullptr, stream));
      }
    }
    XW_HIP(hipEventRecord(sd->fwd, sd->s));
    stream = main_stream;
    XW_HIP(hipStreamWaitEvent((hipStream_t)main_stream, sd->fwd, 0));
  } else {
    XW_ZERO(s->scal, 16);
    if (have_b) {
      XwOdeFwdJob jb = fwd_job(g->xbT, g->start_b, g->ub, g->Yb, g->act_b, g->Nb, 0, (g->narrow >> 1) & 1);
      XW_TRY(xw_ode_fwd_multi(&jb, 1, g->tb, s->theta, s->method, g->Lb, g->d, s->H, s->K, s->m, nullptr, stream));
    }
  }
  if (have_i && !fused_x) {
    XwOdeBwdJob jx = bwd_job(g->xT, g->start, g->Y, g->act, g->N);
    jx.gx = g->gx; jx.gs = g->gs;
    XW_TRY(xw_ode_bwd_multi(&jx, 1, g->t, s->theta, s->method, g->L, g->d, s->H, s->K, s->m, 1 | adj | (((g->narrow >> 5) & 1) ? 16 : 0),
                            stream));
  }
  {
    XwOdeBwdJob jobs[3];
    int nj = 0;
    if (have_i) {
      jobs[nj] = bwd_job(g->xT, g->start, g->Y, g->act, g->N);
      jobs[nj].gslab = g->slabA;
      if (fused_x) { jobs[nj].gx = g->gx; jobs[nj].gs = g->gs; }
      jobs[nj].res_u = g->u; jobs[nj].res_ref = g->pair_i ? g->href : g->h; jobs[nj].res_first_only = 1;
      jobs[nj].res_coef = 2.0 * s->alpha / g->Nglob; jobs[nj].res_base = s->pollution;
      ++nj;
    }
    XwOdeBwdJob jb = bwd_job(g->xbT, g->start_b, g->Yb, g->act_b, g->Nb);
    if (have_b) {
      jb.gslab = g->slabA + (long)g->ns_u * s->Pu;
      jb.res_u = g->ub; jb.res_ref = g->g; jb.res_first_only = 0;
      jb.res_coef = 2.0 * s->alpha / (g->Nbglob * g->Lb); jb.res_base = 0.0;
    }
    if (joint) jobs[nj++] = jb;
    if (have_i) {
      XwOdeBwdJob jB = bwd_job(g->xT, g->start, g->Y, g->act, g->N);
      jB.gslab = g->slabB;
      jB.res_first_only = 2; jB.res_u = g->u; jB.res_ref = g->v;
      jB.res_coef = g->Vol / g->Nglob / g->L * g->s3_scale; jB.res_base = g->Vol / g->Nglob;
      jB.res_w_per_point = g->w_per_point; jB.res_w = g->w; jB.res_c = g->c; jB.res_cp = g->cp; jB.res_kappa2 = 2.0 * g->ckappa;
      jobs[nj++] = jB;
      const int modeA = (fused_x ? (1 | 2 | 4) : 2) | adj | (((g->narrow >> 2) & 1) ? 16 : 0);
      XW_TRY(xw_ode_bwd_multi(jobs, nj, g->t, s->theta, s->method, g->L, g->d, s->H, s->K, s->m, modeA, stream));
    }
    if (have_b && !joint)
      XW_TRY(xw_ode_bwd_multi(&jb, 1, g->tb, s->theta, s->method, g->Lb, g->d, s->H, s->K, s->m, 2 | adj | (((g->narrow >> 3) & 1) ? 16 : 0),
                              stream));
  }
  if (have_i) {
    XW_TRY(contract(g, s, s->step_u, true, !shard, stream));
  } else if (have_b) {
    XW_TRY(xw_bdry_partials(g->ub, g->g, g->Nb, g->Lb, s->alpha, g->Nbglob, nullptr, g->work_b, s->scal, stream));
  }
  if (!shard) {
    XW_TRY(xw_adam(s->theta, g->slabA, g->ns_u + g->ns_b, accum, g->slabB, g->ns_u, nullptr, s->scal, s->m_u, s->v_u, s->step_u, -1, s->Pu,
                   s->lr_u, s->beta1, s->beta2, s->eps, s->grad_u, s->lag_lo, s->lag_hi, adam_skip_field, s->lag_u, stream));
  } else {
    const int nA = (have_i ? g->ns_u : 0) + (have_b ? g->ns_b : 0), nB = have_i ? g->ns_u : 0;
    double* const pA = s->pack_u;
    double* const pB = s->pack_u + s->Pu;
    if (nA > 0 && nB > 0) {
      XW_TRY(xw_slab_sum2(g->slabA, nA, pA, g->slabB, nB, pB, s->Pu, stream));
    } else {
      if (nA > 0) { XW_TRY(xw_slab_sum(g->slabA + (have_i ? 0 : (long)g->ns_u * s->Pu), nA, s->Pu, 0, pA, stream)); } else { XW_ZERO(pA, s->Pu); }
      XW_ZERO(pB, s->Pu);
    }
    XW_TRY(s->exchange(s->pack_u, 2 * s->Pu + 16, s->exchange_ctx, stream));
// ... 73 lines not shown
```

### xnode_wan_pde_solver_amd/csrc/xw_tdopri.hip

```cpp
#include "xw_common.h"
#include "xnwan.h"

namespace {
#include "xw_tiled_blocks.h"
#include "xw_generic_cot.h"

__device__ __forceinline__ double gsum64(double x) { return xw_sum_over_g(xw_sum_over_n(x)); }

#include "xw_dopri_ctl.h"

struct TdWork {
  TileWork w;
  long k, total;
};
__host__ __device__ inline TdWork td_work(int sweep, int d, int H, int K, int m) {
  TdWork q;
  q.w = tile_work(sweep, d, H, K, m);
  q.k = q.w.total;
  q.total = q.w.total + 16L * H * (sweep ? 14 : 7);
  return q;
}

__device__ __forceinline__ void tload(int H, int N, int p0, const double* __restrict__ src, double* v) {
  for (int e = lane_id(); e < 16 * H; e += 64) {
// ... 344 lines not shown
    touter(slab, n.o.Win, n.o.ldin, K, d, Sx, ws + w.xt, A_PLAIN);
  }
  if (want_x && job.gx != nullptr) {
    double* gxt = ws + w.xt + 16L * d;
    tgemm(theta + n.o.Win, 1, n.o.ldin, d, K, Sx, A_PLAIN, nullptr, nullptr, 0, 0.0, nullptr, E_NONE, nullptr, gxt);
    for (int e = lane_id(); e < 16 * d; e += 64)
      if (p0 + (e & 15) < N) job.gx[(long)(e >> 4) * N + p0 + (e & 15)] = gxt[e];
  }
}

bool dims_ok(int d, int H, int K, int m) { return xw_tiled_ode_ok(d, H, K, m) != 0; }

int fwd_check(int njobs, const double* t, const double* theta, int L, int d, int H, int K, int m, int Hn, double rtol, double atol,
              const double* work) {
  if (!t || !theta || !work || L < 1 || njobs < 1 || njobs > XW_DOPRI_MAXJOBS || !(rtol >= 0.0) || !(atol >= 0.0)) return XW_E_ARG;
  if (!dims_ok(d, H, K, m)) return XW_E_DIMS;
  if (Hn < 1 || Hn > H) return XW_E_ARG;
  return 0;
}

int fwd_jobs(const XwDopriJob* jobs, int njobs, Jobs<XwDopriJob>& P) {
  const int e = pack_jobs(jobs, njobs, P);
  if (e) return e;
  for (int i = 0; i < njobs; ++i) {
    const XwDopriJob& j = jobs[i];
    if (!j.xT || !j.start || !j.u || !j.rec_y || !j.rec_t || !j.rec_h || !j.fbuf || !j.ctl || !j.work || j.N < 1 || j.cap < 0)
      return XW_E_ARG;
    P.blk0[i + 1] = P.blk0[i] + (j.N + 15) / 16;
  }
  return 0;
}
}

extern "C" int xw_tdopri5_work(int sweep, int d, int H, int K, int m) {
  if (!dims_ok(d, H, K, m)) return XW_E_DIMS;
  return (int)td_work(sweep != 0, d, H, K, m).total;
}

extern "C" int xw_tdopri5_part_size(int N) { return N < 1 ? XW_E_ARG : 2 * ((N + 15) / 16); }

extern "C" int xw_tdopri5_init(const XwDopriJob* jobs, int njobs, const double* t, const double* theta, int L, int d, int H, int K,
                               int m, int Hn, double rtol, double atol, double* work, void* stream) {
  int e = fwd_check(njobs, t, theta, L, d, H, K, m, Hn, rtol, atol, work);
  if (e) return e;
  Jobs<XwDopriJob> P;
  e = fwd_jobs(jobs, njobs, P);
  if (e) return e;
  hipStream_t s = (hipStream_t)stream;
  const dim3 g(P.blk0[njobs]), b(64);
  hipLaunchKernelGGL(kq_init1, g, b, 0, s, P, t, theta, L, d, H, K, m, Hn, rtol, atol, work);
  hipLaunchKernelGGL(kq_init2, g, b, 0, s, P, t, theta, L, d, H, K, m, Hn, rtol, atol, work);
  return xw_launch_status();
}

extern "C" int xw_tdopri5_attempts(const XwDopriJob* jobs, int njobs, const double* t, const double* theta, int L, int d, int H,
                                   int K, int m, int Hn, double rtol, double atol, int max_steps, int n, double* work,
                                   void* stream) {
  int e = fwd_check(njobs, t, theta, L, d, H, K, m, Hn, rtol, atol, work);
  if (e) return e;
  if (max_steps < 1 || n < 0) return XW_E_ARG;
  Jobs<XwDopriJob> P;
  e = fwd_jobs(jobs, njobs, P);
  if (e) return e;
  hipStream_t s = (hipStream_t)stream;
  const dim3 g(P.blk0[njobs]), b(64);
  for (int i = 0; i < n; ++i)
    hipLaunchKernelGGL(kq_attempt, g, b, 0, s, P, t, theta, L, d, H, K, m, Hn, rtol, atol, max_steps, work);
  return xw_launch_status();
}

extern "C" int xw_tdopri5_sweep(const XwDopriSweepJob* jobs, int njobs, const double* t, const double* theta, int L, int d, int H,
                                int K, int m, int mode, double* work, void* stream) {
  if (!t || !theta || !work || L < 1 || njobs < 1 || njobs > XW_DOPRI_MAXJOBS) return XW_E_ARG;
  if ((mode & 3) == 0 || (mode & ~31) || ((mode & 4) && (mode & 3) != 3)) return XW_E_ARG;
  if (!dims_ok(d, H, K, m) || (mode & (8 | 16))) return XW_E_DIMS;
  Jobs<XwDopriSweepJob> P;
  const int e = pack_jobs(jobs, njobs, P);
  if (e) return e;
  hipStream_t s = (hipStream_t)stream;
  const long Pu = u_offsets(d, H, K).total;
  for (int i = 0; i < njobs; ++i) {
    const XwDopriSweepJob& j = jobs[i];
    if (!j.b.xT || !j.b.start || !j.rec_y || !j.rec_t || !j.rec_h || !j.ctl || j.b.N < 1) return XW_E_ARG;
    if (j.b.res_u != nullptr && j.b.ubar != nullptr) return XW_E_ARG;
    if ((mode & 2) && !j.b.gslab) return XW_E_ARG;
    if ((mode & 1) && !(mode & 4) && (!j.b.gx || !j.b.gs)) return XW_E_ARG;
    P.blk0[i + 1] = P.blk0[i] + (j.b.N + 15) / 16;
  }
  if (mode & 2)
    for (int i = 0; i < njobs; ++i) {
      const hipError_t he = hipMemsetAsync(jobs[i].b.gslab, 0, sizeof(double) * Pu * ((jobs[i].b.N + 15) / 16), s);
      if (he != hipSuccess) return (int)he;
    }
  hipLaunchKernelGGL(kq_sweep, dim3(P.blk0[njobs]), dim3(64), 0, s, P, t, theta, L, d, H, K, m, mode, work);
  return xw_launch_status();
}
```

### xnode_wan_pde_solver_amd/csrc/xw_tiled.hip

```cpp
#include "xw_common.h"
#include "xnwan.h"

namespace {
#include "xw_tiled_blocks.h"

#define XWA_HIST 11

struct AbRows { double b[XWA_HIST + 1][XWA_HIST]; };
__host__ __device__ constexpr AbRows ab_rows() {
  AbRows r{};
  for (int k = 1; k <= XWA_HIST; ++k)
    for (int j = 0; j < k; ++j) {
      long long c[XWA_HIST + 1] = {1};
      int deg = 0;
      for (int i = 0; i < k; ++i) {
        if (i == j) continue;
        for (int p = deg + 1; p >= 1; --p) c[p] = c[p - 1] + (long long)i * c[p];
        c[0] *= i;
        ++deg;
      }
      long long num = 0, den = 27720;
      for (int p = 0; p <= deg; ++p) num += c[p] * (27720 / (p + 1));
      for (int i = 2; i <= j; ++i) den *= i;
      for (int i = 2; i <= k - 1 - j; ++i) den *= i;
// ... 383 lines not shown
      touter(slab, n.o.IL2w, H, H, H, dh2, p0v, A_RELU);
      trowsum(slab, n.o.IL4b, 1, H, l0, nullptr, 1.0);
      trowsum(slab, n.o.IL2b, 1, H, dh2, nullptr, 1.0);
      trowsum(slab, n.o.IL0w, 1, H, dh1, st, 1.0);
      trowsum(slab, n.o.IL0b, 1, H, dh1, nullptr, 1.0);
      sync_tile();
    } else if (lane_id() < 16 && lane_active) {
      double s = 0.0;
      for (int i = 0; i < H; ++i) s = fma(theta[n.o.IL0w + i], dh1[i * 16 + l16], s);
      job.gs[p0 + l16] = s;
    }
  }
  if (slab) {
    trowsum(slab, n.o.Winb, 1, K, Sx, nullptr, 1.0);
    touter(slab, n.o.Win, n.o.ldin, K, d, Sx, ws + w.xt, A_PLAIN);
  }
  if (want_x && job.gx != nullptr) {
    double* gxt = ws + w.xt + 16L * d;
    tgemm(theta + n.o.Win, 1, n.o.ldin, d, K, Sx, A_PLAIN, nullptr, nullptr, 0, 0.0, nullptr, E_NONE, nullptr, gxt);
    for (int e = lane_id(); e < 16 * d; e += 64)
      if (p0 + (e & 15) < N) job.gx[(long)(e >> 4) * N + p0 + (e & 15)] = gxt[e];
  }
}

}

extern "C" int xw_tiled_ode_ok(int d, int H, int K, int m) {
  return H >= 1 && H <= XWT_MAX_H && K >= 1 && K <= XWT_MAX_K && m >= 1 && m <= XWT_MAX_M && d >= 1 && d + 2 <= 128;
}

static long tile_stride(bool ab, int sweep, int d, int H, int K, int m) {
  return tile_work(sweep != 0, d, H, K, m).total + (ab ? 16L * H * (XWA_HIST + (sweep ? 1 : 0)) : 0);
}

extern "C" int xw_tiled_ode_work(int sweep, int d, int H, int K, int m) {
  if (!xw_tiled_ode_ok(d, H, K, m)) return XW_E_DIMS;
  return (int)tile_work(sweep != 0, d, H, K, m).total;
}

extern "C" int xw_tiled_ode_bwd_slabs(int N) { return (N + 15) / 16; }

static int check_common(int njobs, const double* t, const double* theta, int method, int L, int d, int H, int K, int m,
                        const double* work) {
  if (njobs < 1 || !t || !theta || !work || L < 1 || method < 0 || method > 2) return XW_E_ARG;
  if (!xw_tiled_ode_ok(d, H, K, m)) return XW_E_DIMS;
  return 0;
}

static int tiled_fwd(bool ab, const XwOdeFwdJob* jobs, int njobs, const double* t, const double* theta, int method, int L, int d,
                     int H, int K, int m, double* zero16, double* work, void* stream) {
  if (!jobs) return XW_E_ARG;
  const int c = check_common(njobs, t, theta, method, L, d, H, K, m, work);
  if (c) return c;
  hipStream_t s = (hipStream_t)stream;
  for (int i = 0; i < njobs; ++i)
    if (!jobs[i].xT || !jobs[i].start || !jobs[i].u || jobs[i].N < 1) return XW_E_ARG;
  if (zero16 != nullptr) {
    const hipError_t e = hipMemsetAsync(zero16, 0, 16 * sizeof(double), s);
    if (e != hipSuccess) return (int)e;
  }
  const long per = tile_stride(ab, 0, d, H, K, m);
  long off = 0;
  for (int i = 0; i < njobs; ++i) {
    const int tiles = (jobs[i].N + 15) / 16;
    if (ab) hipLaunchKernelGGL(kt_adams_fwd, dim3(tiles), dim3(64), 0, s, jobs[i], t, theta, L, d, H, K, m, work + off);
    else hipLaunchKernelGGL(kt_ode_fwd, dim3(tiles), dim3(64), 0, s, jobs[i], t, theta, method, L, d, H, K, m, work + off);
    off += per * tiles;
  }
  return xw_launch_status();
}

static int tiled_bwd(bool ab, const XwOdeBwdJob* jobs, int njobs, const double* t, const double* theta, int method, int L, int d,
                     int H, int K, int m, int mode, double* work, void* stream) {
  if (!jobs || (mode & 3) == 0) return XW_E_ARG;
  const int c = check_common(njobs, t, theta, method, L, d, H, K, m, work);
  if (c) return c;
  if (mode & (8 | 16)) return XW_E_DIMS;
  if ((mode & 4) && (mode & 3) != 3) return XW_E_ARG;
  hipStream_t s = (hipStream_t)stream;
  const long P = u_offsets(d, H, K).total;
  for (int i = 0; i < njobs; ++i) {
    const XwOdeBwdJob& j = jobs[i];
    if (!j.xT || !j.start || !j.Y || j.N < 1) return XW_E_ARG;
    if (j.res_u != nullptr && j.ubar != nullptr) return XW_E_ARG;
    if ((mode & 2) && !j.gslab) return XW_E_ARG;
    if ((mode & 1) && !(mode & 4) && (!j.gx || !j.gs)) return XW_E_ARG;
  }
  const long per = tile_stride(ab, 1, d, H, K, m);
  long off = 0;
  for (int i = 0; i < njobs; ++i) {
    const XwOdeBwdJob& j = jobs[i];
    const int tiles = (j.N + 15) / 16;
    if (mode & 2) {
      const hipError_t e = hipMemsetAsync(j.gslab, 0, sizeof(double) * P * tiles, s);
      if (e != hipSuccess) return (int)e;
    }
    if (ab) hipLaunchKernelGGL(kt_adams_bwd, dim3(tiles), dim3(64), 0, s, j, t, theta, L, d, H, K, m, mode, work + off);
    else hipLaunchKernelGGL(kt_ode_bwd, dim3(tiles), dim3(64), 0, s, j, t, theta, method, L, d, H, K, m, mode, work + off);
    off += per * tiles;
  }
  return xw_launch_status();
}

extern "C" int xw_tiled_ode_fwd_multi(const XwOdeFwdJob* jobs, int njobs, const double* t, const double* theta, int method, int L,
                                      int d, int H, int K, int m, double* zero16, double* work, void* stream) {
  return tiled_fwd(false, jobs, njobs, t, theta, method, L, d, H, K, m, zero16, work, stream);
}

extern "C" int xw_tiled_ode_bwd_multi(const XwOdeBwdJob* jobs, int njobs, const double* t, const double* theta, int method, int L,
                                      int d, int H, int K, int m, int mode, double* work, void* stream) {
  return tiled_bwd(false, jobs, njobs, t, theta, method, L, d, H, K, m, mode, work, stream);
}

extern "C" int xw_adams_coef(int k, double* out) {
  if (k < 1 || k > XWA_HIST || !out) return XW_E_ARG;
  for (int j = 0; j < k; ++j) out[j] = kABhost.b[k][j];
  return 0;
}

extern "C" int xw_adams_tiled_work(int sweep, int d, int H, int K, int m) {
  if (!xw_tiled_ode_ok(d, H, K, m)) return XW_E_DIMS;
  return (int)tile_stride(true, sweep, d, H, K, m);
}

extern "C" int xw_adams_tiled_fwd_multi(const XwOdeFwdJob* jobs, int njobs, const double* t, const double* theta, int L, int d, int H,
                                        int K, int m, double* zero16, double* work, void* stream) {
  return tiled_fwd(true, jobs, njobs, t, theta, 2, L, d, H, K, m, zero16, work, stream);
}

extern "C" int xw_adams_tiled_bwd_multi(const XwOdeBwdJob* jobs, int njobs, const double* t, const double* theta, int L, int d, int H,
                                        int K, int m, int mode, double* work, void* stream) {
  return tiled_bwd(true, jobs, njobs, t, theta, 2, L, d, H, K, m, mode, work, stream);
}
```

### xnode_wan_pde_solver_amd/engine.py

```python
import contextlib
import math
import os

import torch

from . import kernels as KN
from ._lib import XnwanError
from .options import EngineOptions
from .sampling import HIP_HOST_LOCK, _PIN_POOL, Hypercube, _paths


def ctypes_addr(fn):
    import ctypes
    return ctypes.cast(fn, ctypes.c_void_p).value

_KEPT_GRAPHS = []

_NOSTREAM = contextlib.nullcontext()

_SCRATCH_POOL = []


_DEVICE_STREAMS = {}

# ... 91 lines not shown
        if self.dopri5 and world is not None:
            raise XnwanError("solver 'dopri5' runs on one GPU: its step sizes are per group and chosen on the device, and a "
                             "group sharded over %d ranks would need an exchange per attempted step (not built)" % world.size)
        self.adjoint = bool(config.get('adjoint', False))
        self.alpha = float(config['alpha'])
        self.pollution = 1.0
        self.verify_structure = opt.verify_structure
        self.packed_load = opt.packed_load
        self.refill_variants = 8
        self.verify_every = 16
        sp = setup.get('shape_param', [-1, 1])
        lo, hi = (sp[0], sp[1]) if isinstance(sp, (list, tuple)) else (-sp, sp)
        self.structure = structure if structure is not None else Structure(funcs, self.d, lo, hi)
        if u_mod.blob is None or v_mod.blob is None:
            raise XnwanError('bind() the networks to the device before building the engine')
        (self.H, self.K), self.m = u_mod.kdims, config['u_layers']
        self.W, self.q = v_mod.kwidth, config['v_layers']
        self.stepper = KN.stepper_family(config['u_hidden_dim'], config['u_hidden_hidden_dim'], self.m, opt.tiled_stepper, self.method)
        self.tiled = self.stepper == 'tiled'
        if self.method == KN.ADAMS and self.adjoint:
            from .nets import ADAMS_ADJOINT_REFUSED
            raise XnwanError(ADAMS_ADJOINT_REFUSED)
        if self.tiled:
            if (self.H, self.K) != (config['u_hidden_dim'], config['u_hidden_hidden_dim']):
                raise XnwanError('the tiled stepper family reads theta at the network\'s own widths; the module was bound at %s'
                                 % ((self.H, self.K),))
            if self.adjoint:
                raise XnwanError('adjoint=True (the continuous adjoint) is not served by the tiled stepper family (u_hidden_dim = %d, '
                                 'u_hidden_hidden_dim = %d, u_layers = %d: it reverses the steps taken; the continuous adjoint exists '
                                 'for the MFMA containers %s, u_layers <= %d)' % (self.H, self.K, self.m, KN.ODE_WIDTHS, KN.ODE_MAX_DEPTH))
            if self.dopri5 and self.dopri5_stepper != 'tiled':
                raise XnwanError("solver 'dopri5' is not served by the tiled stepper family (u_hidden_dim = %d, u_hidden_hidden_dim = %d, "
                                 "u_layers = %d): its field code is the generic path's, up to %s and u_layers %d; the tiled family runs "
                                 "the fixed-grid solvers %s -- unless EngineOptions.dopri5_stepper = 'tiled' (XW_DOPRI5_STEPPER) selects "
                                 "dopri5's implementation on that family" % (self.H, self.K, self.m, KN.GENERIC_ODE_MAX,
                                                                              KN.GENERIC_ODE_MAX_DEPTH, sorted(KN.METHODS)))
        self.testnet = getattr(v_mod, 'family', None) or KN.testnet_family(config['v_hidden_dim'], self.q)
        self.testnet_tiled = self.testnet == 'tiled'
        if self.testnet_tiled and self.W != config['v_hidden_dim']:
            raise XnwanError('the tiled test-network family reads phi at the network\'s own width; the module was bound at %d' % self.W)
        self.generic = (self.stepper == 'generic', not self.testnet_tiled and KN.disc_generic(self.W))
        if any(self.generic):
            import warnings
            which = ' and '.join(n_ for n_, g_ in zip(('u_theta (u_hidden_dim %d, u_hidden_hidden_dim %d, u_layers %d)' % (self.H, self.K, self.m),
                                                       'v_phi (v_hidden_dim %d)' % self.W), self.generic) if g_)
            warnings.warn('%s is outside the MFMA kernel instantiations %s (u_layers <= 10) / %s: running on the generic vector-ALU path, expect a step '
                          'rate lower by two to three orders of magnitude' % (which, KN.ODE_WIDTHS, KN.DISC_WIDTHS), RuntimeWarning, stacklevel=3)
        self.xproj_min_d = 1 << 30 if (self.generic[1] or self.testnet_tiled) else int(opt.xproj_min_d)
        if self.W > 64 and not self.generic[1] and not self.testnet_tiled:
            self.xproj_min_d = 0
        if self.generic[0] and self.adjoint:
            raise XnwanError('adjoint=True (the continuous adjoint) exists for the MFMA stepper instantiations %s only; u_hidden_dim = %d, '
                             'u_hidden_hidden_dim = %d run on the generic path, which reverses the steps taken (adjoint=False)'
                             % (KN.ODE_WIDTHS, self.H, self.K))
        self.theta, self.phi = u_mod.blob, v_mod.blob
        self.Pu, self.Pv = self.theta.data.numel(), self.phi.data.numel()
        z = lambda n: torch.zeros(n, dtype=F64, device=device)
        self.adam_u = dict(m=z(self.Pu), v=z(self.Pu), step=torch.zeros(1, dtype=torch.int64, device=device),
                           lag=torch.zeros(1, dtype=torch.int64, device=device))
        self.pairwise_single_slice = opt.pairwise_single_slice
        self.adam_skips_untouched = opt.adam_skips_untouched
        self.eager_checked = 10 ** 12 if opt.always_check else 256
        self.field_range = (self.theta.slots[6][0], self.theta.slots[-2][0])
        self._field_touched = False
        self.adam_v = dict(m=z(self.Pv), v=z(self.Pv), step=torch.zeros(1, dtype=torch.int64, device=device))
        self.grad_u, self.grad_v = z(self.Pu), z(self.Pv)
        self.pack_u = z(2 * self.Pu + 16)
        self.scal = self.pack_u[2 * self.Pu:]
        self.accum_u = self.accum_v = None
        self.use_streams = opt.use_streams
        self.use_graphs = opt.use_graphs
        self.reuse_test_net = opt.reuse_test_net
        self.keep_activations = opt.keep_activations
        cus = torch.cuda.get_device_properties(device).multi_processor_count
        self.v_blocks = int(opt.v_blocks) or (12 * 2 * cus) // 16
        self.v_blocks_disc = int(opt.v_blocks_disc) or (13 * 2 * cus) // 16
        self.narrow = str(opt.narrow)
        if opt.hw_queues > 4:
            import warnings
            warnings.warn('GPU_MAX_HW_QUEUES=%s: the sub-step schedule is tuned for the runtime default of 4 hardware queues and '
                          'measures ~45 %% slower with more' % opt.hw_queues, RuntimeWarning, stacklevel=2)
        self.early_slab_sum = opt.early_slab_sum
        self.compact_tiles = int(opt.compact_tiles)
        self.prio_drop = {'A': int(opt.prio_drop_A) if opt.prio_drop_A is not None else (3 if self.d <= 32 else 2),
                          'X': int(opt.prio_drop_X), 'F': int(opt.prio_drop_F), 'G': int(opt.prio_drop_G)}
        self.use_runner = opt.use_runner
        if self.dopri5:
            self.use_graphs = self.use_streams = self.use_runner = self.keep_activations = False
        if self.tiled:
            self.use_runner = self.keep_activations = False
            self.narrow = '0'
        if self.testnet_tiled:
            self.use_runner = False
        self.narrow_set = str(opt.narrow_set)
        self.narrow_tiles = {'f': 192, 'x': 128, 'p': 64}
        if opt.narrow_tiles:
            self.narrow_tiles = dict(zip('fxp', (int(v_) for v_ in str(opt.narrow_tiles).split(':'))))
        self.narrow_tiles_alone = dict(zip('fxp', (int(v_) for v_ in str(opt.narrow_tiles_alone).split(':'))))
        for k_ in 'fxp':
            self.narrow_tiles_alone[k_] = max(self.narrow_tiles_alone[k_], self.narrow_tiles[k_])
        self.simds = 4 * cus
        self._phi_version = 0
        self.streams, self._cap = _device_streams(device)
        self.capture_exchange = (world is not None and getattr(world, 'capturable', False)
                                 and opt.capture_exchange)
        if self.capture_exchange:
            world.all_reduce(self.scal)

    def _tabulate_a(self, X1):
        d, dev, fa = self.d, self.dev, self.funcs['a']
        N = X1.shape[0]
        A = None
        try:
            ii = torch.arange(d, device=X1.device).view(d, 1, 1, 1)
            jj = torch.arange(d, device=X1.device).view(1, d, 1, 1)
            out = fa(X1.unsqueeze(0).unsqueeze(0), ii, jj)
            if torch.is_tensor(out) and tuple(out.shape) == (d, d, N, 1):
                A = out[..., 0].to(dev).to(F32).to(F64)
                g = torch.Generator().manual_seed(d * 7919 + N)
                for _ in range(3):
                    i, j = (int(k) for k in torch.randint(0, d, (2,), generator=g))
                    if not torch.equal(A[i, j], fa(X1, i, j).to(dev).to(F32).to(F64)[:, 0]):
                        A = None
                        break
        except Exception:
            A = None
        if A is None:
            A = torch.stack([torch.stack([fa(X1, i, j).to(dev).to(F32).to(F64)[:, 0] for j in range(d)], 0) for i in range(d)], 0)
        off = A.clone()
        off.diagonal(dim1=0, dim2=1).zero_()
        if bool(torch.all(A == A[:, :, :1])):
            return A[:, :, 0].contiguous(), 1
        if bool(torch.all(off == 0)):
            return A.diagonal(dim1=0, dim2=1).t().contiguous(), 2
        return A.contiguous(), 3

    def _tabulate_b(self, X1):
        d, dev, fb = self.d, self.dev, self.funcs['b']
        N = X1.shape[0]
        try:
            out = fb(X1.unsqueeze(0), torch.arange(d, device=X1.device).view(d, 1, 1))
            if torch.is_tensor(out) and tuple(out.shape) == (d, N, 1):
                B = out[..., 0].to(dev).to(F32).to(F64)
                if all(torch.equal(B[i], fb(X1, i).to(dev).to(F32).to(F64)[:, 0]) for i in (0, d // 2, d - 1)):
                    return B.contiguous()
        except Exception:
            pass
        return torch.stack([fb(X1, i).to(dev).to(F32).to(F64)[:, 0] for i in range(d)], 0).contiguous()

    def _check_structure(self, X, version):
        st, d = self.structure, self.d
        X1 = X[:, :1, :]
        bad = []
        if st.a_identity:
            for i in range(d):
                j = (i + 1 + version % max(d - 1, 1)) % d
                bad.append(('func_a[%d,%d] == 1' % (i, i), torch.any(self.funcs['a'](X1, i, i) != 1)))
                if d > 1:
                    bad.append(('func_a[%d,%d] == 0' % (i, j), torch.any(self.funcs['a'](X1, i, j) != 0)))
        if st.b_zero:
            for i in range(d):
                bad.append(('func_b[%d] == 0' % i, torch.any(self.funcs['b'](X1, i) != 0)))
        if st.c_kappa is not None:
            key = (tuple(X.shape[:2]), str(X.device))
            if getattr(self, '_probe_u', (None, None))[0] != key:
                g = torch.Generator().manual_seed(1)
# ... 466 lines not shown
        return torch.cuda.stream(st)

    def _mark(self):
        return torch.cuda.current_stream().record_event() if self.use_streams else None

    def _join(self, *events):
        if self.use_streams:
            cur = torch.cuda.current_stream()
            for ev in events:
                if ev is not None:
                    cur.wait_event(ev)

    def _launch_test_net_here(self, G, blocks=None):
        ph, blocks = self.phi.data, blocks or self.v_blocks
        act = G.vact if getattr(G, 'vact_valid', False) else None
        if G.tpp is not None:
            KN.disc_fwd(G.xvT_pts, None, ph, self.W, self.q, tpp=G.tpp, v=G.v.view(1, -1), vt=G.vt.view(1, -1),
                        gxv=G.gxv, gtv=G.gtv, ngrad=G.N, max_blocks=blocks, act=act)
        else:
            xp = KN.disc_xproj(G.xvT, ph, self.W, out=G.xproj) if 'xproj' in G._lazy else None
            KN.disc_fwd(G.xvT, G.t, ph, self.W, self.q, v=G.v, vt=G.vt, gxv=G.gxv, gtv=G.gtv, ngrad=G.N,
                        max_blocks=blocks, act=act, xproj=xp)

    def _reaction(self, G):
        ck = self.structure.c_kappa
        if ck is None and G.pair_i:
            N = G.N
            ul = G.u.t().detach().requires_grad_(True)
            with torch.enable_grad():
                c = self.funcs['c'](G.X, ul)
                c = c.reshape(N, N) if c.numel() == N * N and N > 1 else c.reshape(-1)
                if c.dim() == 2:
                    if getattr(G, 'sharded', False):
                        raise XnwanError('func_c returns a table over all pairs of paths on a single-slice group (it mixes u [N, 1] with a slice of X that '
                                         'kept its last axis): that needs every path of the group on one rank -- run such groups replicated '
                                         '(XW_REPLICATE_BELOW >= their size) or on one GPU')
                    c = c.mean(0)
                elif c.numel() != N:
                    raise XnwanError('func_c on a single-slice group returned %d values for %d paths' % (c.numel(), N))
                cp = torch.autograd.grad(c.sum(), ul)[0] if c.requires_grad else torch.zeros_like(ul)
            if G.c is None:
                G.c, G.cp = torch.empty_like(G.u), torch.empty_like(G.u)
            G.c.copy_(c.detach().reshape(1, N))
            G.cp.copy_(cp.detach().reshape(1, N))
            ck = 0.0
        elif ck is None:
            ul = G.u.t().unsqueeze(2).detach().requires_grad_(True)
            with torch.enable_grad():
                c = self.funcs['c'](G.X, ul)
                cp = torch.autograd.grad(c.sum(), ul)[0] if c.requires_grad else torch.zeros_like(ul)
            if G.c is None:
                G.c, G.cp = torch.empty_like(G.u), torch.empty_like(G.u)
            G.c.copy_(c.detach().squeeze(2).t())
            G.cp.copy_(cp.detach().squeeze(2).t())
            ck = 0.0
        G.ck = ck

    def _runner_state(self):
        from ._lib import XwSolverState
        st = getattr(self, '_xw_state', None)
        if st is None:
            st = self._xw_state = XwSolverState()
            st.method, st.H, st.K, st.m, st.W, st.q, st.Pu, st.Pv = self.method, self.H, self.K, self.m, self.W, self.q, self.Pu, self.Pv
            st.adjoint = 1 if self.adjoint else 0
            st.lag_lo, st.lag_hi = self.field_range
            st.beta1, st.beta2, st.eps = 0.9, 0.999, 1e-8
            st.theta, st.phi, st.scal = self.theta.data.data_ptr(), self.phi.data.data_ptr(), self.scal.data_ptr()
            st.grad_u, st.grad_v = self.grad_u.data_ptr(), self.grad_v.data_ptr()
            st.m_u, st.v_u, st.m_v, st.v_v = (self.adam_u['m'].data_ptr(), self.adam_u['v'].data_ptr(), self.adam_v['m'].data_ptr(),
                                              self.adam_v['v'].data_ptr())
            st.step_u, st.step_v, st.lag_u = self.adam_u['step'].data_ptr(), self.adam_v['step'].data_ptr(), self.adam_u['lag'].data_ptr()
            st.exchange = st.exchange_ctx = st.pack_u = None
            if self.world is not None:
                st.pack_u = self.pack_u.data_ptr()
                if self.world.comm is not None:
                    from ._lib import lib
                    import ctypes
                    st.exchange = ctypes.cast(lib.xw_allreduce, ctypes.c_void_p).value
                    st.exchange_ctx = self.world.comm.value if hasattr(self.world.comm, 'value') else self.world.comm
                else:
                    self._exchange_cb = self._host_exchange()
                    st.exchange = ctypes_addr(self._exchange_cb)
        st.v_blocks, st.v_blocks_disc = self.v_blocks, self.v_blocks_disc
        st.alpha, st.pollution = float(self.alpha), float(self.pollution)
        st.lr_u, st.lr_v = float(self.config['u_rate']), float(self.config['v_rate'])
        return st

    def _host_exchange(self):
        from ._lib import EXCHANGE_FN
        bufs = {t.data_ptr(): t for t in (self.pack_u, self.scal, self.grad_v)}

        def exchange(buf, count, _ctx, _stream):
            try:
                self.world.all_reduce(bufs[buf][:count])
                return 0
            except BaseException as e:
                self._exchange_error = e
                return -4
        return EXCHANGE_FN(exchange)

    def _runner_group(self, G):
        from ._lib import XwGroup
        xg = getattr(G, '_xw_group', None)
        if xg is None:
            xg = G._xw_group = XwGroup()
            p = lambda t: 0 if t is None else t.data_ptr()
            xg.N, xg.Nb, xg.L, xg.Lb, xg.d = G.N, G.Nb, G.L, G.Lb, self.d
            xg.same_grid, xg.w_per_point, xg.amode = int(bool(G.same_grid)), int(G.w.dim() == 2), int(G.amode)
            xg.ns_u, xg.ns_b = G.ns_u, G.ns_b
            for k in ('xT', 'xvT', 'xbT', 't', 'tb', 'tpp', 'xvT_pts', 'start', 'start_b', 'h', 'href', 'f', 'g', 'w', 'wt', 'w0', 'ghT',
                      'gwx0T', 'A0', 'B0', 'u', 'Y', 'act', 'act_b', 'v', 'vt', 'gxv', 'gtv', 'gx', 'gs', 'vbar', 's3x', 'vact',
                      'xproj', 'slabA', 'slabB', 'slab_v', 'work_i', 'work_b', 'ub', 'Yb'):
                setattr(xg, k, G.ptr(k))
            nar = lambda jobs, **kw: self._narrow_ok(jobs, **kw)
            ji, jb = self._job(G, 'i'), (self._job(G, 'b') if G.Nb else None)
            joint = G.Nb and G.same_grid
            bits = [nar([ji] + ([jb] if joint else []), alone=False, forward=True),
                    bool(jb) and nar([jb], alone=False, forward=True),
                    nar([ji] + ([jb] if joint else []) + [ji], alone=False),
                    bool(jb) and nar([jb], alone=False),
                    False,
                    nar([ji], alone=False, params=False),
                    nar([ji], alone=False, forward=True),
                    nar([ji], alone=False, params=False)]
            xg.narrow = sum(1 << i for i, b in enumerate(bits) if b)
        xg.sharded = int(bool(getattr(G, 'sharded', False)))
        xg.pair_i, xg.pair_b = int(bool(G.pair_i)), int(bool(G.pair_b))
        xg.Vol, xg.Nglob, xg.Nbglob, xg.s3_scale = float(G.Vol), float(G.Nglob), float(G.Nbglob), float(G.s3_scale)
        xg.init_off, xg.bdry_off, xg.ckappa = float(G.init_off), float(G.bdry_off), float(self.structure.c_kappa)
        xg.href = 0 if G.href is None else G.href.data_ptr()
        xg.c = xg.cp = 0
        return xg

    def _runner_ok(self, G):
        return (self.use_runner and self.structure.c_kappa is not None and G.c is None and not getattr(G, 'persistent', True))

    def _world_of(self, G):
        return self.world if getattr(G, 'sharded', self.world is not None) else None

    def _field_seen(self, G):
        touched = G.L > 1 or (getattr(G, 'has_bdry', G.Nb > 0) and G.Lb > 1)
        self._field_touched = touched or (self.accum_u is not None and self._field_touched)
        return self._field_touched

    def _narrow_ok(self, jobs, alone, forward=False, params=True):
        kind = 'f' if forward else ('p' if params else 'x')
        if self.narrow == '0' or kind not in self.narrow_set:
            return False
        if not forward and (self.adjoint or self.method > 1 or any(j.get('act') is None for j in jobs)):
            return False
        if self.narrow == '2':
            return True
        tiles = sum((j['xT'].shape[1] + 15) // 16 for j in jobs)
        return tiles <= (self.narrow_tiles_alone if alone else self.narrow_tiles)[kind]

    def _job(self, G, which, ubar=None, gslab=None, want_x=False):
        if which == 'i':
            j = dict(xT=G.xT, start=G.start, u=G.u, Y=G.Y, act=G.act, ubar=ubar, gslab=gslab)
            if want_x:
                j.update(gx=G.gx, gs=G.gs)
        else:
            j = dict(xT=G.xbT, start=G.start_b, u=G.ub, Y=G.Yb, act=G.act_b, ubar=ubar, gslab=gslab)
        return j

    def _contract(self, G, adam_state=None, with_bdry=False):
        fin = None
        if self._world_of(G) is None and adam_state is not None:
            fin = dict(Lb=G.Lb, Nbglob=G.Nbglob, alpha=self.alpha, step=adam_state['step'], init_off=G.init_off, bdry_off=G.bdry_off)
        pair = dict(href=G.href, s3_scale=G.s3_scale) if G.pair_i else None
        bdry = dict(ub=G.ub, g=G.g) if (with_bdry and G.Nb) else None
        if G.A0 is None and G.B0 is None:
            KN.weak_partials(G.u, G.v, G.vt, G.w, G.f, G.h, G.Vol, G.Nglob, self.scal, G.work_i, c=G.c, ckappa=G.ck, wt=G.wt,
                             contract=dict(gx=G.gx, gs=G.gs, ghT=G.ghT, gxv=G.gxv, w0=G.w0, gwx0T=G.gwx0T), finalize=fin, pair=pair,
                             bdry=bdry)
            return
        KN.weak_contract_general(G.A0, G.amode, G.B0, G.gx, G.gs, G.ghT, G.gxv, G.w0, G.gwx0T, G.v[0], G.s3x)
        KN.weak_partials(G.u, G.v, G.vt, G.w, G.f, G.h, G.Vol, G.Nglob, self.scal, G.work_i, s3x=G.s3x, c=G.c, ckappa=G.ck,
                         wt=G.wt, finalize=fin, pair=pair, bdry=bdry)

    def _gen_all(self, G):
        self._gen_front(G)
        self._gen_back(G)

    def _gen_front(self, G):
        th = self.theta.data
        M = (self.method, self.H, self.K, self.m)
        e0 = self._mark()
        fused_x = self.pollution == 1.0 and not self.adjoint
        joint = G.Nb and G.same_grid
        e_x = None
        if self._compact(G, fused_x, joint):
            return self._gen_front_compact(G)
        if not getattr(G, 'skip_v', False):
            self._launch_test_net_here(G)
        with self._side(1, e0):
            fwd = [self._job(G, 'i')] + ([self._job(G, 'b')] if joint else [])
            self._ode_fwd_multi(fwd, G.t, th, *M, zero16=self.scal, narrow=self._narrow_ok(fwd, alone=False, forward=True),
                             prio_drop=self.prio_drop['G'])
            if G.Nb and not joint:
                fwd_b = [self._job(G, 'b')]
                self._ode_fwd_multi(fwd_b, G.tb, th, *M, narrow=self._narrow_ok(fwd_b, alone=False, forward=True))
            self._reaction(G)
            e_f = self._mark()
            res_A = dict(u=G.u, ref=G.href if G.pair_i else G.h, coef=2.0 * self.alpha / G.Nglob, base=self.pollution, first_only=True)
            res_b = dict(u=G.ub, ref=G.g, coef=2.0 * self.alpha / (G.Nbglob * G.Lb), base=0.0, first_only=False) if G.Nb else None
            e_b = None
            if not fused_x:
                with self._side(2, e_f):
                    sweep_x = [self._job(G, 'i', want_x=True)]
                    self._ode_bwd_multi(sweep_x, G.t, th, *M, want_x=True, want_params=False, adjoint=self.adjoint,
                                     narrow=self._narrow_ok(sweep_x, alone=False, params=False))
                    e_x = self._mark()
            sweeps = [dict(self._job(G, 'i', None, G.slabA[:G.ns_u], want_x=fused_x), res=res_A)]
            if joint:
                sweeps.append(dict(self._job(G, 'b', None, G.slabA[G.ns_u:]), res=res_b))
            self._ode_bwd_multi(sweeps, G.t, th, *M, want_x=fused_x, want_params=True, x_cot_ones=fused_x, adjoint=self.adjoint,
                             narrow=self._narrow_ok(sweeps, alone=False), prio_drop=self.prio_drop['A'])
            if G.Nb and not joint:
                sweep_b = [dict(self._job(G, 'b', None, G.slabA[G.ns_u:]), res=res_b)]
                self._ode_bwd_multi(sweep_b, G.tb, th, *M, want_x=False, want_params=True, adjoint=self.adjoint,
                                 narrow=self._narrow_ok(sweep_b, alone=False))
            e_A = self._mark()
            G.sumA_ready = self.early_slab_sum and self._world_of(G) is None and self.accum_u is None and self.use_streams
            e_S = None
            if G.sumA_ready:
                if getattr(G, 'sumA', None) is None:
                    G.sumA = torch.empty(self.Pu, dtype=F64, device=self.dev)
                KN.slab_sum(G.slabA, out=G.sumA)
                e_S = self._mark()
        e_v = self._mark()
        self._join(e_f)
        res_B = dict(u=G.u, ref=G.v, coef=G.Vol / G.Nglob / G.L * G.s3_scale, base=G.Vol / G.Nglob,
                     weak=dict(w=G.w, c=G.c, cp=G.cp, ckappa=G.ck))
        sweep_B = [dict(self._job(G, 'i', None, G.slabB), res=res_B)]
        self._ode_bwd_multi(sweep_B, G.t, th, *M, want_x=False, want_params=True, adjoint=self.adjoint,
                         narrow=self._narrow_ok(sweep_B, alone=True))
        with self._side(3, e_A, e_v, *[e for e in (e_x, e_b) if e is not None]):
            self._contract(G, self.adam_u, with_bdry=True)
            e_C = self._mark()
        self._join(e_C, e_S)

    def _compact(self, G, fused_x, joint):
        tiles = (G.N + 15) // 16 + ((G.Nb + 15) // 16 if G.Nb else 0)
        if not (self.compact_tiles > 0 and self.use_streams and fused_x and joint):
            return False
        return tiles <= self.compact_tiles or bool(getattr(G, 'skip_v', False))

    def _gen_front_compact(self, G):
        th = self.theta.data
        M = (self.method, self.H, self.K, self.m)
        e0 = self._mark()
        if not getattr(G, 'skip_v', False):
            self._launch_test_net_here(G)
        with self._side(1, e0):
            fwd = [self._job(G, 'i'), self._job(G, 'b')]
            lone = bool(getattr(G, 'skip_v', False))
            self._ode_fwd_multi(fwd, G.t, th, *M, zero16=self.scal, narrow=self._narrow_ok(fwd, alone=lone, forward=True),
                             prio_drop=self.prio_drop['G'])
            self._reaction(G)
            e_f = self._mark()
        self._join(e_f)
        res_A = dict(u=G.u, ref=G.href if G.pair_i else G.h, coef=2.0 * self.alpha / G.Nglob, base=self.pollution, first_only=True)
        res_b = dict(u=G.ub, ref=G.g, coef=2.0 * self.alpha / (G.Nbglob * G.Lb), base=0.0, first_only=False)
        res_B = dict(u=G.u, ref=G.v, coef=G.Vol / G.Nglob / G.L * G.s3_scale, base=G.Vol / G.Nglob,
                     weak=dict(w=G.w, c=G.c, cp=G.cp, ckappa=G.ck))
        sweeps = [dict(self._job(G, 'i', None, G.slabA[:G.ns_u], want_x=True), res=res_A),
                  dict(self._job(G, 'b', None, G.slabA[G.ns_u:]), res=res_b),
                  dict(self._job(G, 'i', None, G.slabB), res=res_B)]
        self._ode_bwd_multi(sweeps, G.t, th, *M, want_x=True, want_params=True, x_cot_ones=True, adjoint=self.adjoint,
                         narrow=self._narrow_ok(sweeps, alone=bool(getattr(G, 'skip_v', False))))
        G.sumA_ready = False
        self._contract(G, self.adam_u, with_bdry=True)

    def begin_substep(self, which, accumulate):
        name, P = ('accum_u', self.Pu) if which == 'u' else ('accum_v', self.Pv)
        if which == 'u':
            self._field_touched = False
        if not accumulate:
            setattr(self, name, None)
        elif getattr(self, name) is None:
            setattr(self, name, torch.zeros(P, dtype=F64, device=self.dev))
        else:
            getattr(self, name).zero_()

    def _gen_back(self, G):
        lr, st = self.config['u_rate'], self.adam_u
        acc = self.accum_u
        world = self._world_of(G)
        lag = dict(lag=st['lag'], lag_range=self.field_range, skip=self.adam_skips_untouched and not self._field_seen(G))
        if world is not None:
            if G.pair_i:
                KN.pair_fold(self.scal, G.Vol, G.Nglob)
            KN.losses(self.scal, G.L, G.Lb, G.Vol, G.Nglob, G.Nbglob, self.alpha, step=st['step'], init_off=G.init_off,
                      bdry_off=G.bdry_off)
        if world is None and getattr(G, 'sumA_ready', False) and acc is None:
            KN.adam(self.theta.data, None, st['m'], st['v'], st['step'], lr, gslabB=G.slabB, scal=self.scal,
                    gextraA=G.sumA, gsum_out=self.grad_u, bump_step=-1, **lag)
        elif world is None:
            KN.adam(self.theta.data, G.slabA, st['m'], st['v'], st['step'], lr, gslabB=G.slabB, scal=self.scal,
                    gextraA=acc, gsum_out=self.grad_u, bump_step=-1, **lag)
        else:
            P = self.Pu
            if acc is not None:
                self.pack_u[:P].add_(acc)
            KN.adam(self.theta.data, None, st['m'], st['v'], st['step'], lr, gextraA=self.pack_u[:P],
                    gextraB=self.pack_u[P:2 * P], scal=self.scal, gsum_out=self.grad_u, bump_step=-1, **lag)
        if acc is not None:
            acc.copy_(self.grad_u)

    def _v_fresh(self, G, store=False):
        now = self._v_key(G)
        G.skip_v = self.reuse_test_net and getattr(G, 'v_version', None) == now
        G.v_version = now
        if not G.skip_v:
            G.vact_valid = G.vact is not None and (store or self.reuse_test_net)
        return ('_vcached' if G.skip_v else '') + ('_act' if getattr(G, 'vact_valid', False) else '')

    def _v_key(self, G):
        return (self._phi_version, sum(p._version for p in self.phi.params), G.sample_version)

    def invalidate_test_net(self):
        self._phi_version += 1

    def _run_runner(self, fn, *args):
        from ._lib import check
        self._exchange_error = None
        rc = fn(*args)
        if getattr(self, '_exchange_error', None) is not None:
            err, self._exchange_error = self._exchange_error, None
            raise err
        check(rc, fn.__name__)

    def generator_step(self, G):
        sfx = self._v_fresh(G)
        world = self._world_of(G)
        if self._runner_ok(G):
            from ._lib import lib
            skip = self.adam_skips_untouched and not self._field_seen(G)
            G.ck = self.structure.c_kappa
            self._run_runner(lib.xw_substep_gen, self._runner_group(G), self._runner_state(), int(bool(G.skip_v)),
                             int(bool(getattr(G, 'vact_valid', False))), KN._p(self.accum_u), int(skip), KN._stream())
            return
        if world is None:
            self._run(G, 'gen' + sfx, self._gen_all)
            return
        if self.capture_exchange:
            self._run(G, 'gen_dist' + sfx, self._gen_all_dist)
            return
        self._run(G, 'gen_front' + sfx, self._gen_front_packed)
        world.all_reduce(self.pack_u)
        self._run(G, 'gen_back', self._gen_back)

    def _gen_all_dist(self, G):
        self._gen_front_packed(G)
        self.world.all_reduce(self.pack_u)
        self._gen_back(G)

    def _gen_front_packed(self, G):
        P = self.Pu
        if G.N == 0:
            return self._gen_front_empty(G)
        self._gen_front(G)
        KN.slab_sum2(G.slabA, self.pack_u[:P], G.slabB, self.pack_u[P:2 * P])

    def _gen_front_empty(self, G):
        P, th = self.Pu, self.theta.data
        M = (self.method, self.H, self.K, self.m)
        self.pack_u.zero_()
        if not G.Nb:
            return
        fwd_b = [self._job(G, 'b')]
        self._ode_fwd_multi(fwd_b, G.tb, th, *M, narrow=self._narrow_ok(fwd_b, alone=False, forward=True))
        res_b = dict(u=G.ub, ref=G.g, coef=2.0 * self.alpha / (G.Nbglob * G.Lb), base=0.0, first_only=False)
        sweep_b = [dict(self._job(G, 'b', None, G.slabA[G.ns_u:]), res=res_b)]
        self._ode_bwd_multi(sweep_b, G.tb, th, *M, want_x=False, want_params=True, adjoint=self.adjoint,
                         narrow=self._narrow_ok(sweep_b, alone=False))
        KN.bdry_partials(G.ub, G.g, self.alpha, G.Nbglob, self.scal, G.work_b)
        KN.slab_sum(G.slabA[G.ns_u:], out=self.pack_u[:P])
# ... 195 lines not shown
```

### xnode_wan_pde_solver_amd/kernels.py

```python
import torch

from ._lib import lib, check, XnwanError, XwOdeFwdJob, XwOdeBwdJob, XwDopriJob, XwDopriSweepJob

METHODS = {'euler': 0, 'midpoint': 1, 'rk4': 2}
DOPRI5 = 3
ADAMS = 4
ADAPTIVE_REFUSED = ('dopri8', 'bosh3', 'fehlberg2', 'adaptive_heun', 'adams', 'implicit_adams',
                    'fixed_adams', 'scipy_solver')
F32, F64 = torch.float32, torch.float64


def _need_gpu():
    if not torch.cuda.is_available():
        raise XnwanError('no GPU visible: the XNODE-WAN kernels only run on an MI355X (gfx950); there is no CPU path')


TRUSTED = False
LONE_NARROW = __import__('os').environ.get('XW_LONE_NARROW', '1') == '1'


def _chk(t, dtype, shape, name):
    if t is None or TRUSTED:
        return
    if not (torch.is_tensor(t) and t.is_cuda):
# ... 108 lines not shown
    if not (1 <= W <= TILED_DISC_MAX and 0 <= q <= TILED_DISC_MAX_DEPTH):
        raise XnwanError('v_hidden_dim = %d, v_layers = %d: the test-network kernels serve widths up to %d (MFMA containers %s) / %d '
                         '(generic path) / %d (tiled), depths up to %d / %d / %d'
                         % (W, q, DISC_WIDTHS[-1], DISC_WIDTHS, GENERIC_DISC_MAX, TILED_DISC_MAX, DISC_MAX_GRAD_DEPTH,
                            DISC_MAX_GRAD_DEPTH, TILED_DISC_MAX_DEPTH))
    return 'mfma' if W <= GENERIC_DISC_MAX and q <= DISC_MAX_GRAD_DEPTH else 'tiled'


def testnet_kwidth(W, q):
    return disc_container(W) if testnet_family(W, q) == 'mfma' else W


def _disc_family(W, q, family):
    if family is None:
        return testnet_family(W, q)
    if family not in TESTNET_FAMILIES:
        raise XnwanError('family = %r: one of %s' % (family, TESTNET_FAMILIES))
    return family


def theta_size(d, H, K):
    return lib.xw_theta_size(d, H, K)


def phi_size(d, W):
    return lib.xw_phi_size(d, W)


def ode_fwd(xT, t, start, theta, method, H, K, m, want_Y=True, u=None, Y=None):
    _need_gpu()
    d, N = xT.shape
    L = t.shape[0]
    _chk(xT, F64, (d, N), 'xT'); _chk(t, F64, (L,), 't'); _chk(start, F64, (N,), 'start')
    _chk(theta, F64, (theta_size(d, H, K),), 'theta')
    if u is None:
        u = torch.empty(L, N, dtype=F64, device=xT.device)
    if Y is None and want_Y:
        Y = torch.empty(L, H, N, dtype=F64, device=xT.device)
    _chk(u, F64, (L, N), 'u'); _chk(Y, F64, (L, H, N), 'Y')
    if Y is None and LONE_NARROW and (N + 15) // 16 <= 256 and (H, K) in ODE_WIDTHS:
        arr = (XwOdeFwdJob * 1)()
        a = arr[0]
        a.xT, a.start, a.u, a.Y, a.act, a.N, a.act_x_only, a.narrow, a.prio_drop = _p(xT), _p(start), _p(u), 0, 0, N, 0, 1, 0
        check(lib.xw_ode_fwd_multi(arr, 1, _p(t), _p(theta), method, L, d, H, K, m, 0, _stream()), 'xw_ode_fwd_multi')
        return u, None
    check(lib.xw_ode_fwd(_p(xT), _p(t), _p(start), _p(theta), method, N, L, d, H, K, m, _p(u), _p(Y), _stream()), 'xw_ode_fwd')
    return u, Y


def ode_fwd_multi(jobs, t, theta, method, H, K, m, zero16=None, act_x_only=False, narrow=False, prio_drop=0):
    _need_gpu()
    L = t.shape[0]
    d = jobs[0]['xT'].shape[0]
    _chk(t, F64, (L,), 't'); _chk(theta, F64, (theta_size(d, H, K),), 'theta')
    arr = (XwOdeFwdJob * len(jobs))()
    for a, j in zip(arr, jobs):
        N = j['xT'].shape[1]
        _chk(j['xT'], F64, (d, N), 'xT'); _chk(j['start'], F64, (N,), 'start'); _chk(j['u'], F64, (L, N), 'u')
        _chk(j.get('Y'), F64, (L, H, N), 'Y')
        if j.get('act') is not None:
            _chk(j['act'], F64, (max(L - 1, 1), ode_act_rows(method, H, K, m), ode_act_cols(N)), 'act')
        a.xT, a.start, a.u, a.Y, a.act, a.N = _p(j['xT']), _p(j['start']), _p(j['u']), _p(j.get('Y')), _p(j.get('act')), N
        a.act_x_only = 1 if act_x_only else 0
        a.narrow = 1 if narrow else 0
        a.prio_drop = int(prio_drop)
    _chk(zero16, F64, (16,), 'zero16')
    check(lib.xw_ode_fwd_multi(arr, len(jobs), _p(t), _p(theta), method, L, d, H, K, m, _p(zero16), _stream()), 'xw_ode_fwd_multi')


def _set_res(a, j, L, N):
    res = j.get('res')
    if res is not None:
        if j.get('ubar') is not None:
            raise XnwanError('a sweep job takes a stored cotangent (ubar) or a residual (res), not both')
        if res.get('weak') is not None:
            wk = res['weak']
            wpp = wk['w'].dim() == 2
            _chk(res['u'], F64, (L, N), 'res.u'); _chk(res['ref'], F64, (L, N), 'res.ref (v)')
            _chk(wk['w'], F64, (L, N) if wpp else (N,), 'res.weak.w'); _chk(wk.get('c'), F64, (L, N), 'res.weak.c')
            _chk(wk.get('cp'), F64, (L, N), 'res.weak.cp')
            a.res_first_only, a.res_u, a.res_ref = 2, _p(res['u']), _p(res['ref'])
            a.res_w_per_point, a.res_w, a.res_c, a.res_cp = int(wpp), _p(wk['w']), _p(wk.get('c')), _p(wk.get('cp'))
            a.res_kappa2 = 2.0 * float(wk.get('ckappa', 0.0))
        else:
            first = bool(res['first_only'])
            _chk(res['u'], F64, (L, N), 'res.u'); _chk(res['ref'], F64, (N,) if first else (L, N), 'res.ref')
            a.res_first_only, a.res_u, a.res_ref = int(first), _p(res['u']), _p(res['ref'])
        a.res_coef, a.res_base = float(res['coef']), float(res['base'])


def ode_bwd_multi(jobs, t, theta, method, H, K, m, want_x, want_params, x_cot_ones=False, adjoint=False, narrow=False, prio_drop=0):
    _need_gpu()
    L = t.shape[0]
    d = jobs[0]['xT'].shape[0]
    P = theta_size(d, H, K)
    _chk(t, F64, (L,), 't'); _chk(theta, F64, (P,), 'theta')
    arr = (XwOdeBwdJob * len(jobs))()
    for a, j in zip(arr, jobs):
        N = j['xT'].shape[1]
        _chk(j['xT'], F64, (d, N), 'xT'); _chk(j['start'], F64, (N,), 'start'); _chk(j['Y'], F64, (L, H, N), 'Y')
        _chk(j.get('ubar'), F64, (L, N), 'ubar')
        if want_x and not (x_cot_ones and j.get('gx') is None):
            _chk(j['gx'], F64, (d, N), 'gx'); _chk(j['gs'], F64, (N,), 'gs')
        if want_params:
            _chk(j['gslab'], F64, (ode_bwd_slabs(N), P), 'gslab')
        if j.get('act') is not None:
            _chk(j['act'], F64, (max(L - 1, 1), ode_act_rows(method, H, K, m), ode_act_cols(N)), 'act')
        a.xT, a.start, a.Y, a.ubar, a.N = _p(j['xT']), _p(j['start']), _p(j['Y']), _p(j.get('ubar')), N
        a.act = _p(j.get('act'))
        a.gx, a.gs, a.gslab = _p(j.get('gx')), _p(j.get('gs')), _p(j.get('gslab'))
        _set_res(a, j, L, N)
    if x_cot_ones and not (want_x and want_params):
        raise XnwanError('x_cot_ones needs want_x and want_params')
    if x_cot_ones and adjoint:
        raise XnwanError('x_cot_ones is not available with the continuous adjoint')
    if narrow and (adjoint or method > 1 or any(j.get('act') is None for j in jobs)):
        raise XnwanError('narrow-tile sweeps run from the activation store of euler / midpoint (no adjoint=True, no rk4)')
    mode = (1 if want_x else 0) | (2 if want_params else 0) | (4 if x_cot_ones else 0) | (8 if adjoint else 0) | (16 if narrow else 0) | ((int(prio_drop) & 3) << 5)
    check(lib.xw_ode_bwd_multi(arr, len(jobs), _p(t), _p(theta), method, L, d, H, K, m, mode, _stream()), 'xw_ode_bwd_multi')


def tiled_ode_work(sweep, d, H, K, m, tiles, dev, method=None):
    per = (lib.xw_adams_tiled_work if method == ADAMS else lib.xw_tiled_ode_work)(1 if sweep else 0, d, H, K, m)
    check(min(per, 0), 'xw_tiled_ode_work')
    return torch.empty(per * tiles, dtype=F64, device=dev)


def tiled_ode_fwd_multi(jobs, t, theta, method, H, K, m, zero16=None, prio_drop=0, **_hints):
    if method == ADAMS:
        return adams_tiled_fwd_multi(jobs, t, theta, H, K, m, zero16=zero16, prio_drop=prio_drop)
    _tiled_fwd(jobs, t, theta, method, H, K, m, zero16, prio_drop)


def adams_tiled_fwd_multi(jobs, t, theta, H, K, m, zero16=None, prio_drop=0, **_hints):
    _tiled_fwd(jobs, t, theta, ADAMS, H, K, m, zero16, prio_drop)


def _tiled_fwd(jobs, t, theta, method, H, K, m, zero16, prio_drop):
    _need_gpu()
    L = t.shape[0]
    d = jobs[0]['xT'].shape[0]
    _chk(t, F64, (L,), 't'); _chk(theta, F64, (theta_size(d, H, K),), 'theta')
    if method != ADAMS and method not in METHODS.values():
        raise XnwanError("the tiled stepper family runs the fixed-grid methods %s and 'explicit_adams' only" % sorted(METHODS))
    arr = (XwOdeFwdJob * len(jobs))()
    for a, j in zip(arr, jobs):
        N = j['xT'].shape[1]
        _chk(j['xT'], F64, (d, N), 'xT'); _chk(j['start'], F64, (N,), 'start'); _chk(j['u'], F64, (L, N), 'u')
        _chk(j.get('Y'), F64, (L, H, N), 'Y')
        a.xT, a.start, a.u, a.Y, a.act, a.N = _p(j['xT']), _p(j['start']), _p(j['u']), _p(j.get('Y')), 0, N
        a.act_x_only, a.narrow, a.prio_drop = 0, 0, int(prio_drop)
    _chk(zero16, F64, (16,), 'zero16')
    work = tiled_ode_work(False, d, H, K, m, sum(lib.xw_tiled_ode_bwd_slabs(a.N) for a in arr), t.device, method)
    if method == ADAMS:
        check(lib.xw_adams_tiled_fwd_multi(arr, len(jobs), _p(t), _p(theta), L, d, H, K, m, _p(zero16), _p(work), _stream()),
              'xw_adams_tiled_fwd_multi')
    else:
        check(lib.xw_tiled_ode_fwd_multi(arr, len(jobs), _p(t), _p(theta), method, L, d, H, K, m, _p(zero16), _p(work), _stream()),
              'xw_tiled_ode_fwd_multi')


def tiled_ode_bwd_multi(jobs, t, theta, method, H, K, m, want_x, want_params, x_cot_ones=False, adjoint=False, narrow=False,
                        prio_drop=0):
    if method == ADAMS:
        return adams_tiled_bwd_multi(jobs, t, theta, H, K, m, want_x, want_params, x_cot_ones=x_cot_ones, adjoint=adjoint,
                                     narrow=narrow, prio_drop=prio_drop)
# ... 565 lines not shown
```

### xnode_wan_pde_solver_amd/options.py

```python
import dataclasses
import os
from typing import Optional


def _flag(name, default):
    v = os.environ.get(name)
    if v is None:
        return default
    return v != '0' if default else v == '1'


def _int(name, default):
    v = os.environ.get(name)
    return default if v in (None, '') else int(v)


@dataclasses.dataclass
class EngineOptions:
    use_streams: bool = True
    use_graphs: bool = True
    strict_graphs: bool = False
    reuse_test_net: bool = False
    keep_activations: bool = True
    v_blocks: int = 0
    v_blocks_disc: int = 0
    narrow: str = '1'
    narrow_set: str = 'fx'
    narrow_tiles: Optional[str] = None
    narrow_tiles_alone: str = '256:256:64'
    early_slab_sum: bool = True
    compact_tiles: int = 320
    prio_drop_A: Optional[int] = None
    prio_drop_X: int = 0
    prio_drop_F: int = 0
    prio_drop_G: int = 0
    use_runner: bool = True
    capture_exchange: bool = True
    xproj_min_d: int = 45
    tiled_stepper: str = 'beyond'
    hw_queues: int = 4
    verify_structure: bool = True
    packed_load: bool = True
    pairwise_single_slice: bool = True
    adam_skips_untouched: bool = True
    always_check: bool = False
    poison: bool = False
    capture_refill: bool = True
    defer_list_readback: bool = True
    sampler_process: bool = True
    show_plan: bool = False
    dopri5_chunk: int = 8
    dopri5_max_steps: int = 10000
    dopri5_stepper: str = 'vector'
    replicate_below: int = 16
    native_allreduce: bool = True

    @classmethod
    def from_env(cls):
        o = cls()
        o.use_streams = _flag('XW_STREAMS', o.use_streams)
        o.use_graphs = _flag('XW_GRAPHS', o.use_graphs)
        o.strict_graphs = _flag('XW_STRICT_GRAPHS', o.strict_graphs)
        o.reuse_test_net = _flag('XW_REUSE_V', o.reuse_test_net)
        o.keep_activations = _flag('XW_KEEP_ACT', o.keep_activations)
        o.v_blocks = _int('XW_V_BLOCKS', o.v_blocks)
        o.v_blocks_disc = _int('XW_V_BLOCKS_DISC', o.v_blocks_disc)
        o.narrow = os.environ.get('XW_NARROW', o.narrow)
        o.narrow_set = os.environ.get('XW_NARROW_SET', o.narrow_set)
        o.narrow_tiles = os.environ.get('XW_NARROW_TILES') or None
        o.narrow_tiles_alone = os.environ.get('XW_NARROW_TILES_ALONE') or o.narrow_tiles_alone
        o.early_slab_sum = _flag('XW_EARLY_SLAB_SUM', o.early_slab_sum)
        o.compact_tiles = _int('XW_COMPACT_TILES', o.compact_tiles)
        o.prio_drop_A = _int('XW_PRIO_DROP_A', None)
        o.prio_drop_X = _int('XW_PRIO_DROP_X', o.prio_drop_X)
        o.prio_drop_F = _int('XW_PRIO_DROP_F', o.prio_drop_F)
        o.prio_drop_G = _int('XW_PRIO_DROP_G', o.prio_drop_G)
        o.use_runner = _flag('XW_RUNNER', o.use_runner)
        o.capture_exchange = _flag('XW_CAPTURE_EXCHANGE', o.capture_exchange)
        o.xproj_min_d = _int('XW_XPROJ_MIN_D', o.xproj_min_d)
        o.tiled_stepper = os.environ.get('XW_TILED_STEPPER') or o.tiled_stepper
        try:
            o.hw_queues = _int('GPU_MAX_HW_QUEUES', o.hw_queues)
        except ValueError:
            pass
        o.verify_structure = _flag('XW_VERIFY_STRUCTURE', o.verify_structure)
        o.packed_load = _flag('XW_PACKED_LOAD', o.packed_load)
        o.pairwise_single_slice = not _flag('XW_ELEMENTWISE_SINGLE_SLICE', False)
        o.adam_skips_untouched = not _flag('XW_ADAM_NO_SKIP', False)
        o.always_check = _flag('XW_ALWAYS_CHECK', o.always_check)
        o.poison = _flag('XW_POISON', o.poison)
        o.capture_refill = _flag('XW_CAPTURE_REFILL', o.capture_refill)
        o.defer_list_readback = _flag('XW_DEFER_LIST', o.defer_list_readback)
        o.sampler_process = _flag('XW_SAMPLER_PROCESS', o.sampler_process)
        o.show_plan = _flag('XW_SHOW_PLAN', o.show_plan)
        o.dopri5_chunk = _int('XW_DOPRI5_CHUNK', o.dopri5_chunk)
        o.dopri5_max_steps = _int('XW_DOPRI5_MAX_STEPS', o.dopri5_max_steps)
        o.dopri5_stepper = os.environ.get('XW_DOPRI5_STEPPER') or o.dopri5_stepper
        o.replicate_below = _int('XW_REPLICATE_BELOW', o.replicate_below)
        o.native_allreduce = _flag('XW_NATIVE_ALLREDUCE', o.native_allreduce)
        return o

    def non_default(self):
        base = EngineOptions()
        return {f.name: getattr(self, f.name) for f in dataclasses.fields(self) if getattr(self, f.name) != getattr(base, f.name)}
```

Before: 2126.

## Merge interior adjoint cotangent sweeps into one backward parameter pass

Adds a merged cotangent mode (res_first_only=3) that folds the initial-condition residual term, scaled by 2/scal[0], into the weak-form cotangent. This lets the interior generator substep run one backward parameter sweep instead of separate A and B slab sweeps, and Adam then reads a single slab. The aim is to remove a full backward ODE sweep and the slab summation per substep. In exchange the sweep must wait for the contraction that produces scal, which serialises work that previously overlapped.

```diff
diff --git a/include/xnwan.h b/include/xnwan.h
--- a/include/xnwan.h
+++ b/include/xnwan.h
@@ -38,6 +38,7 @@
                  double* gx; double* gs; double* gslab; int N;
                  int res_first_only; const double* res_u; const double* res_ref; double res_coef; double res_base;
                  int res_w_per_point; const double* res_w; const double* res_c; const double* res_cp; double res_kappa2;
+                 const double* res_scal; const double* res_refA; double res_coefA; double res_baseA;
                } XwOdeBwdJob;
 int xw_ode_bwd_multi(const XwOdeBwdJob* jobs, int njobs, const double* t, const double* theta,
                      int method, int L, int d, int H, int K, int m, int mode, void* stream);
@@ -163,6 +164,7 @@
   XwExchangeFn exchange;
   void* exchange_ctx;
   double* pack_u;
+  int merged_sweep;
 } XwSolverState;
 int xw_substep_gen(const XwGroup* g, const XwSolverState* s, int skip_v, int store_record, double* accum, int adam_skip_field,
                    void* stream);
diff --git a/xnode_wan_pde_solver_amd/_lib.py b/xnode_wan_pde_solver_amd/_lib.py
--- a/xnode_wan_pde_solver_amd/_lib.py
+++ b/xnode_wan_pde_solver_amd/_lib.py
@@ -20,7 +20,8 @@
     _fields_ = [('xT', c_vp), ('start', c_vp), ('Y', c_vp), ('act', c_vp), ('ubar', c_vp), ('gx', c_vp), ('gs', c_vp),
                 ('gslab', c_vp), ('N', c_int), ('res_first_only', c_int), ('res_u', c_vp), ('res_ref', c_vp),
                 ('res_coef', ctypes.c_double), ('res_base', ctypes.c_double), ('res_w_per_point', c_int), ('res_w', c_vp),
-                ('res_c', c_vp), ('res_cp', c_vp), ('res_kappa2', ctypes.c_double)]
+                ('res_c', c_vp), ('res_cp', c_vp), ('res_kappa2', ctypes.c_double), ('res_scal', c_vp), ('res_refA', c_vp),
+                ('res_coefA', ctypes.c_double), ('res_baseA', ctypes.c_double)]
 
 
 class XwDopriJob(ctypes.Structure):
@@ -47,7 +48,8 @@
                                       'lag_hi')]
                 + [(n, c_dbl) for n in ('alpha', 'pollution', 'lr_u', 'lr_v', 'beta1', 'beta2', 'eps')]
                 + [(n, c_vp) for n in ('theta', 'phi', 'scal', 'grad_u', 'grad_v', 'm_u', 'v_u', 'm_v', 'v_v', 'step_u', 'step_v',
-                                       'lag_u', 'exchange', 'exchange_ctx', 'pack_u')])
+                                       'lag_u', 'exchange', 'exchange_ctx', 'pack_u')]
+                + [('merged_sweep', c_int)])
 
 
 EXCHANGE_FN = ctypes.CFUNCTYPE(ctypes.c_int, ctypes.c_void_p, ctypes.c_int, ctypes.c_void_p, ctypes.c_void_p)
diff --git a/xnode_wan_pde_solver_amd/csrc/xw_common.h b/xnode_wan_pde_solver_amd/csrc/xw_common.h
--- a/xnode_wan_pde_solver_amd/csrc/xw_common.h
+++ b/xnode_wan_pde_solver_amd/csrc/xw_common.h
@@ -58,6 +58,15 @@
 __device__ __forceinline__ void xw_st_g(double v, double* p) { *(xw_gp)p = v; }
 __device__ __forceinline__ double xw_ld_nt(const double* p) { return __builtin_nontemporal_load((xw_gcp)p); }
 __device__ __forceinline__ void xw_st_nt(double v, double* p) { __builtin_nontemporal_store(v, (xw_gp)p); }
+
+__device__ __forceinline__ double xw_cot_init(double base, double coef, double u, double ref, bool first) {
+  return first ? fma(coef, u - ref, base) : base;
+}
+__device__ __forceinline__ double xw_cot_weak(double coef, double base, double dcu, double v, double w, bool last) {
+  const double g = coef * dcu * v * w;
+  return last ? fma(base, v, g) : g;
+}
+__device__ __forceinline__ double xw_cot_merged(double a, double s, double b) { return fma(s, b, a); }
 
 __device__ __forceinline__ int xw_lane() { return threadIdx.x & 63; }
 
diff --git a/xnode_wan_pde_solver_amd/csrc/xw_dopri.hip b/xnode_wan_pde_solver_amd/csrc/xw_dopri.hip
--- a/xnode_wan_pde_solver_amd/csrc/xw_dopri.hip
+++ b/xnode_wan_pde_solver_amd/csrc/xw_dopri.hip
@@ -408,7 +408,7 @@
   for (int i = 0; i < njobs; ++i) {
     const XwDopriSweepJob& j = jobs[i];
     if (!j.b.xT || !j.b.start || !j.rec_y || !j.rec_t || !j.rec_h || !j.ctl || j.b.N < 1) return XW_E_ARG;
-    if (j.b.res_u != nullptr && j.b.ubar != nullptr) return XW_E_ARG;
+    if (!cot_job_ok(j.b)) return XW_E_ARG;
     if ((mode & 2) && !j.b.gslab) return XW_E_ARG;
     if ((mode & 1) && !(mode & 4) && (!j.b.gx || !j.b.gs)) return XW_E_ARG;
     if (mode & 2) {
diff --git a/xnode_wan_pde_solver_amd/csrc/xw_generic.hip b/xnode_wan_pde_solver_amd/csrc/xw_generic.hip
--- a/xnode_wan_pde_solver_amd/csrc/xw_generic.hip
+++ b/xnode_wan_pde_solver_amd/csrc/xw_generic.hip
@@ -400,7 +400,7 @@
   for (int i = 0; i < njobs; ++i) {
     const XwOdeBwdJob& j = jobs[i];
     if (!j.xT || !j.start || !j.Y || j.N < 1) return XW_E_ARG;
-    if (j.res_u != nullptr && j.ubar != nullptr) return XW_E_ARG;
+    if (!cot_job_ok(j)) return XW_E_ARG;
     if ((mode & 2) && !j.gslab) return XW_E_ARG;
     if ((mode & 1) && !(mode & 4) && (!j.gx || !j.gs)) return XW_E_ARG;
     if (mode & 2) {
diff --git a/xnode_wan_pde_solver_amd/csrc/xw_generic_cot.h b/xnode_wan_pde_solver_amd/csrc/xw_generic_cot.h
--- a/xnode_wan_pde_solver_amd/csrc/xw_generic_cot.h
+++ b/xnode_wan_pde_solver_amd/csrc/xw_generic_cot.h
@@ -1,15 +1,25 @@
 #pragma once
+__device__ __forceinline__ double cot_weak(const XwOdeBwdJob& j, int l, int L, int path, long p) {
+  const double u = j.res_u[p], v = j.res_ref[p];
+  const double w = j.res_w_per_point ? j.res_w[p] : j.res_w[path];
+  const double dcu = j.res_c != nullptr ? j.res_c[p] + u * j.res_cp[p] : j.res_kappa2 * u;
+  return xw_cot_weak(j.res_coef, j.res_base, dcu, v, w, l == L - 1);
+}
 __device__ double cot_u(const XwOdeBwdJob& j, int l, int L, int path) {
   const long p = (long)l * j.N + path;
   if (j.res_u == nullptr) return j.ubar ? j.ubar[p] : 1.0;
-  if (j.res_first_only == 2) {
-    const double u = j.res_u[p], v = j.res_ref[p];
-    const double w = j.res_w_per_point ? j.res_w[p] : j.res_w[path];
-    const double dcu = j.res_c != nullptr ? j.res_c[p] + u * j.res_cp[p] : j.res_kappa2 * u;
-    double g = j.res_coef * dcu * v * w;
-    if (l == L - 1) g += j.res_base * v;
-    return g;
-  }
-  if (j.res_first_only == 1) return l == 0 ? j.res_base + j.res_coef * (j.res_u[p] - j.res_ref[path]) : j.res_base;
+  if (j.res_first_only == 3)
+    return xw_cot_merged(xw_cot_init(j.res_baseA, j.res_coefA, j.res_u[p], j.res_refA[path], l == 0), 2.0 / j.res_scal[0],
+                         cot_weak(j, l, L, path, p));
+  if (j.res_first_only == 2) return cot_weak(j, l, L, path, p);
+  if (j.res_first_only == 1) return xw_cot_init(j.res_base, j.res_coef, j.res_u[p], j.res_ref[path], l == 0);
   return j.res_base + j.res_coef * (j.res_u[p] - j.res_ref[p]);
 }
+inline bool cot_job_ok(const XwOdeBwdJob& j) {
+  if (j.res_first_only < 0 || j.res_first_only > 3) return false;
+  if (j.res_u == nullptr) return j.res_first_only != 3;
+  if (j.ubar != nullptr || j.res_ref == nullptr) return false;
+  if (j.res_first_only >= 2 && (j.res_w == nullptr || (!j.res_c != !j.res_cp))) return false;
+  if (j.res_first_only == 3 && (j.res_scal == nullptr || j.res_refA == nullptr)) return false;
+  return true;
+}
diff --git a/xnode_wan_pde_solver_amd/csrc/xw_ode.hip b/xnode_wan_pde_solver_amd/csrc/xw_ode.hip
--- a/xnode_wan_pde_solver_amd/csrc/xw_ode.hip
+++ b/xnode_wan_pde_solver_amd/csrc/xw_ode.hip
@@ -285,43 +285,49 @@
   const double* res_cp[XW_MAXJOBS];
   double res_kappa2[XW_MAXJOBS];
   int res_wpp[XW_MAXJOBS];
+  const double* res_scal[XW_MAXJOBS];
+  const double* res_refA[XW_MAXJOBS];
+  double res_coefA[XW_MAXJOBS], res_baseA[XW_MAXJOBS];
 };
 __device__ __forceinline__ double cot_u(const BwdJobs& jobs, int job, const double* __restrict__ ubar, int l, int N, int col,
                                         int L) {
   const double* __restrict__ ru = jobs.res_u[job];
   if (ru != nullptr) {
-    if (jobs.res_first[job] == 2) {
+    if (jobs.res_first[job] >= 2) {
       const long p = (long)l * N + col;
       const double ul = ru[p], vl = jobs.res_ref[job][p];
       const double wl = jobs.res_wpp[job] ? jobs.res_w[job][p] : jobs.res_w[job][col];
       const double dcu = jobs.res_c[job] != nullptr ? jobs.res_c[job][p] + ul * jobs.res_cp[job][p] : jobs.res_kappa2[job] * ul;
-      double gB = jobs.res_coef[job] * dcu * vl * wl;
-      if (l == L - 1) gB += jobs.res_base[job] * vl;
-      return gB;
-    }
+      const double gB = xw_cot_weak(jobs.res_coef[job], jobs.res_base[job], dcu, vl, wl, l == L - 1);
+      if (jobs.res_first[job] == 2) return gB;
+      return xw_cot_merged(xw_cot_init(jobs.res_baseA[job], jobs.res_coefA[job], ul, jobs.res_refA[job][col], l == 0),
+                           2.0 / jobs.res_scal[job][0], gB);
+    }
+    if (jobs.res_first[job]) return xw_cot_init(jobs.res_base[job], jobs.res_coef[job], ru[col], jobs.res_ref[job][col], l == 0);
     double r = jobs.res_base[job];
-    if (jobs.res_first[job]) {
-      if (l == 0) r += jobs.res_coef[job] * (ru[col] - jobs.res_ref[job][col]);
-    } else {
-      r += jobs.res_coef[job] * (ru[(long)l * N + col] - jobs.res_ref[job][(long)l * N + col]);
-    }
+    r += jobs.res_coef[job] * (ru[(long)l * N + col] - jobs.res_ref[job][(long)l * N + col]);
     return r;
   }
   return ubar != nullptr ? ubar[(long)l * N + col] : 1.0;
 }
 struct Cot4 {
-  const double *p0, *p1, *p2, *p3, *p4;
+  const double *p0, *p1, *p2, *p3, *p4, *p5;
   long s0, s1, s2;
-  double cb, coef, base, kappa2;
-  bool weak, use_st, use_res, first, tab, valid;
-};
-struct CotRaw { double a, b, c, d, e; };
+  double cb, coef, base, kappa2, s, coefA, baseA;
+  bool weak, use_st, use_res, first, tab, valid, merged;
+};
+struct CotRaw { double a, b, c, d, e, f; };
 __device__ __forceinline__ Cot4 make_cot(const BwdJobs& jobs, int job, int N, int col, bool valid, const double* dummy) {
   Cot4 c;
   const double* ru = jobs.res_u[job];
   const double* ubar = jobs.ubar[job];
   c.valid = valid;
-  c.weak = ru != nullptr && jobs.res_first[job] == 2;
+  c.weak = ru != nullptr && jobs.res_first[job] >= 2;
+  c.merged = ru != nullptr && jobs.res_first[job] == 3;
+  c.coefA = jobs.res_coefA[job];
+  c.baseA = jobs.res_baseA[job];
+  c.s = 2.0 / xw_ld_g(c.merged ? jobs.res_scal[job] : dummy);
+  c.p5 = (c.merged ? jobs.res_refA[job] : dummy) + col;
   c.use_res = ru != nullptr && !c.weak;
   c.use_st = ru == nullptr && ubar != nullptr;
   c.first = c.use_res && jobs.res_first[job] != 0;
@@ -350,9 +356,10 @@
     r.c = xw_ld_g(c.p2 + l * c.s2);
     r.d = xw_ld_g(c.p3 + l * c.s1);
     r.e = xw_ld_g(c.p4 + l * c.s1);
+    r.f = xw_ld_g(c.p5);
   } else {
     r.c = xw_ld_g(c.p2 + l * c.s1);
-    r.d = r.e = 0.0;
+    r.d = r.e = r.f = 0.0;
   }
   return r;
 }
@@ -360,12 +367,14 @@
   double ub;
   if (WEAK) {
     const double dcu = c.tab ? fma(r.a, r.e, r.d) : c.kappa2 * r.a;
-    ub = c.coef * dcu * r.b * r.c;
-    if (l == L - 1) ub = fma(c.base, r.b, ub);
+    ub = xw_cot_weak(c.coef, c.base, dcu, r.b, r.c, l == L - 1);
+    if (c.merged) ub = xw_cot_merged(xw_cot_init(c.baseA, c.coefA, r.a, r.f, l == 0), c.s, ub);
+  } else if (c.first) {
+    ub = xw_cot_init(c.cb, c.coef, r.b, r.c, l == 0);
   } else {
     ub = c.cb;
     if (c.use_st) ub += r.a;
-    if (c.use_res && (!c.first || l == 0)) ub = fma(c.coef, r.b - r.c, ub);
+    if (c.use_res) ub = fma(c.coef, r.b - r.c, ub);
   }
   return c.valid ? ub : 0.0;
 }
@@ -1214,9 +1223,14 @@
     J.res_cp[i] = on ? jobs[i].res_cp : nullptr;
     J.res_kappa2[i] = on ? jobs[i].res_kappa2 : 0.0;
     J.res_wpp[i] = on ? jobs[i].res_w_per_point : 0;
+    J.res_scal[i] = on ? jobs[i].res_scal : nullptr;
+    J.res_refA[i] = on ? jobs[i].res_refA : nullptr;
+    J.res_coefA[i] = on ? jobs[i].res_coefA : 0.0;
+    J.res_baseA[i] = on ? jobs[i].res_baseA : 0.0;
     if (on && jobs[i].res_u && (!jobs[i].res_ref || jobs[i].ubar)) return XW_E_ARG;
-    if (on && jobs[i].res_u && jobs[i].res_first_only == 2 && (!jobs[i].res_w || (!jobs[i].res_c != !jobs[i].res_cp))) return XW_E_ARG;
-    if (on && (jobs[i].res_first_only < 0 || jobs[i].res_first_only > 2)) return XW_E_ARG;
+    if (on && jobs[i].res_u && jobs[i].res_first_only >= 2 && (!jobs[i].res_w || (!jobs[i].res_c != !jobs[i].res_cp))) return XW_E_ARG;
+    if (on && (jobs[i].res_first_only < 0 || jobs[i].res_first_only > 3)) return XW_E_ARG;
+    if (on && jobs[i].res_first_only == 3 && (!jobs[i].res_u || !jobs[i].res_scal || !jobs[i].res_refA)) return XW_E_ARG;
     J.gx[i] = (on && (mode & 1)) ? jobs[i].gx : nullptr;
     J.gs[i] = (on && (mode & 1)) ? jobs[i].gs : nullptr;
     J.gslab[i] = (on && (mode & 2)) ? jobs[i].gslab : nullptr;
diff --git a/xnode_wan_pde_solver_amd/csrc/xw_substep.hip b/xnode_wan_pde_solver_amd/csrc/xw_substep.hip
--- a/xnode_wan_pde_solver_amd/csrc/xw_substep.hip
+++ b/xnode_wan_pde_solver_amd/csrc/xw_substep.hip
@@ -73,6 +73,43 @@
   const bool joint = have_i && have_b && g->same_grid;
   const int adj = s->adjoint ? 8 : 0;
   void* const main_stream = stream;
+  const bool merged = s->merged_sweep && !shard && accum == nullptr && fused_x && joint && !g->pair_i && !g->pair_b && g->A0 == nullptr &&
+                      g->B0 == nullptr;
+  if (merged) {
+    Side* sd = side_of_current_device();
+    if (sd == nullptr) return XW_E_ARG;
+    XW_HIP(hipEventRecord(sd->fork, (hipStream_t)main_stream));
+    XW_HIP(hipStreamWaitEvent(sd->s, sd->fork, 0));
+    if (!skip_v) XW_TRY(test_net(g, s, s->v_blocks, store_record ? g->vact : nullptr, main_stream));
+    {
+      XwOdeFwdJob jobs[2] = {fwd_job(g->xT, g->start, g->u, g->Y, g->act, g->N, 0, (g->narrow >> 0) & 1),
+                             fwd_job(g->xbT, g->start_b, g->ub, g->Yb, g->act_b, g->Nb, 0, (g->narrow >> 0) & 1)};
+      XW_TRY(xw_ode_fwd_multi(jobs, 2, g->t, s->theta, s->method, g->L, g->d, s->H, s->K, s->m, s->scal, (void*)sd->s));
+      XwOdeBwdJob jx = bwd_job(g->xT, g->start, g->Y, g->act, g->N);
+      jx.gx = g->gx; jx.gs = g->gs;
+      XW_TRY(xw_ode_bwd_multi(&jx, 1, g->t, s->theta, s->method, g->L, g->d, s->H, s->K, s->m, 1 | (((g->narrow >> 5) & 1) ? 16 : 0),
+                              (void*)sd->s));
+    }
+    XW_HIP(hipEventRecord(sd->fwd, sd->s));
+    XW_HIP(hipStreamWaitEvent((hipStream_t)main_stream, sd->fwd, 0));
+    XW_TRY(contract(g, s, s->step_u, true, true, main_stream));
+    XwOdeBwdJob jobs[2];
+    jobs[0] = bwd_job(g->xT, g->start, g->Y, g->act, g->N);
+    jobs[0].gslab = g->slabA;
+    jobs[0].res_first_only = 3; jobs[0].res_u = g->u; jobs[0].res_ref = g->v;
+    jobs[0].res_coef = g->Vol / g->Nglob / g->L * g->s3_scale; jobs[0].res_base = g->Vol / g->Nglob;
+    jobs[0].res_w_per_point = g->w_per_point; jobs[0].res_w = g->w; jobs[0].res_c = g->c; jobs[0].res_cp = g->cp;
+    jobs[0].res_kappa2 = 2.0 * g->ckappa;
+    jobs[0].res_scal = s->scal; jobs[0].res_refA = g->h; jobs[0].res_coefA = 2.0 * s->alpha / g->Nglob; jobs[0].res_baseA = s->pollution;
+    jobs[1] = bwd_job(g->xbT, g->start_b, g->Yb, g->act_b, g->Nb);
+    jobs[1].gslab = g->slabA + (long)g->ns_u * s->Pu;
+    jobs[1].res_u = g->ub; jobs[1].res_ref = g->g; jobs[1].res_first_only = 0;
+    jobs[1].res_coef = 2.0 * s->alpha / (g->Nbglob * g->Lb); jobs[1].res_base = 0.0;
+    XW_TRY(xw_ode_bwd_multi(jobs, 2, g->t, s->theta, s->method, g->L, g->d, s->H, s->K, s->m, 2 | (((g->narrow >> 4) & 1) ? 16 : 0),
+                            main_stream));
+    return xw_adam(s->theta, g->slabA, g->ns_u + g->ns_b, nullptr, nullptr, 0, nullptr, nullptr, s->m_u, s->v_u, s->step_u, -1, s->Pu,
+                   s->lr_u, s->beta1, s->beta2, s->eps, s->grad_u, s->lag_lo, s->lag_hi, adam_skip_field, s->lag_u, main_stream);
+  }
   if (have_i) {
     Side* sd = side_of_current_device();
     if (sd == nullptr) return XW_E_ARG;
diff --git a/xnode_wan_pde_solver_amd/csrc/xw_tdopri.hip b/xnode_wan_pde_solver_amd/csrc/xw_tdopri.hip
--- a/xnode_wan_pde_solver_amd/csrc/xw_tdopri.hip
+++ b/xnode_wan_pde_solver_amd/csrc/xw_tdopri.hip
@@ -450,7 +450,7 @@
   for (int i = 0; i < njobs; ++i) {
     const XwDopriSweepJob& j = jobs[i];
     if (!j.b.xT || !j.b.start || !j.rec_y || !j.rec_t || !j.rec_h || !j.ctl || j.b.N < 1) return XW_E_ARG;
-    if (j.b.res_u != nullptr && j.b.ubar != nullptr) return XW_E_ARG;
+    if (!cot_job_ok(j.b)) return XW_E_ARG;
     if ((mode & 2) && !j.b.gslab) return XW_E_ARG;
     if ((mode & 1) && !(mode & 4) && (!j.b.gx || !j.b.gs)) return XW_E_ARG;
     P.blk0[i + 1] = P.blk0[i] + (j.b.N + 15) / 16;
diff --git a/xnode_wan_pde_solver_amd/csrc/xw_tiled.hip b/xnode_wan_pde_solver_amd/csrc/xw_tiled.hip
--- a/xnode_wan_pde_solver_amd/csrc/xw_tiled.hip
+++ b/xnode_wan_pde_solver_amd/csrc/xw_tiled.hip
@@ -489,7 +489,7 @@
   for (int i = 0; i < njobs; ++i) {
     const XwOdeBwdJob& j = jobs[i];
     if (!j.xT || !j.start || !j.Y || j.N < 1) return XW_E_ARG;
-    if (j.res_u != nullptr && j.ubar != nullptr) return XW_E_ARG;
+    if (!cot_job_ok(j)) return XW_E_ARG;
     if ((mode & 2) && !j.gslab) return XW_E_ARG;
     if ((mode & 1) && !(mode & 4) && (!j.gx || !j.gs)) return XW_E_ARG;
   }
diff --git a/xnode_wan_pde_solver_amd/engine.py b/xnode_wan_pde_solver_amd/engine.py
--- a/xnode_wan_pde_solver_amd/engine.py
+++ b/xnode_wan_pde_solver_amd/engine.py
@@ -197,6 +197,7 @@
                           'measures ~45 %% slower with more' % opt.hw_queues, RuntimeWarning, stacklevel=2)
         self.early_slab_sum = opt.early_slab_sum
         self.compact_tiles = int(opt.compact_tiles)
+        self.merged_sweep = bool(opt.merged_sweep)
         self.prio_drop = {'A': int(opt.prio_drop_A) if opt.prio_drop_A is not None else (3 if self.d <= 32 else 2),
                           'X': int(opt.prio_drop_X), 'F': int(opt.prio_drop_F), 'G': int(opt.prio_drop_G)}
         self.use_runner = opt.use_runner
@@ -829,6 +830,7 @@
                     self._exchange_cb = self._host_exchange()
                     st.exchange = ctypes_addr(self._exchange_cb)
         st.v_blocks, st.v_blocks_disc = self.v_blocks, self.v_blocks_disc
+        st.merged_sweep = int(self.merged_sweep)
         st.alpha, st.pollution = float(self.alpha), float(self.pollution)
         st.lr_u, st.lr_v = float(self.config['u_rate']), float(self.config['v_rate'])
         return st
@@ -866,7 +868,7 @@
                     bool(jb) and nar([jb], alone=False, forward=True),
                     nar([ji] + ([jb] if joint else []) + [ji], alone=False),
                     bool(jb) and nar([jb], alone=False),
-                    False,
+                    bool(joint) and nar([ji, jb], alone=False),
                     nar([ji], alone=False, params=False),
                     nar([ji], alone=False, forward=True),
                     nar([ji], alone=False, params=False)]
@@ -936,6 +938,9 @@
         fused_x = self.pollution == 1.0 and not self.adjoint
         joint = G.Nb and G.same_grid
         e_x = None
+        G.merged = self._merged_ok(G, fused_x, joint)
+        if G.merged:
+            return self._gen_front_merged(G)
         if self._compact(G, fused_x, joint):
             return self._gen_front_compact(G)
         if not getattr(G, 'skip_v', False):
@@ -1019,6 +1024,37 @@
         G.sumA_ready = False
         self._contract(G, self.adam_u, with_bdry=True)
 
+    def _merged_ok(self, G, fused_x, joint):
+        return bool(self.merged_sweep and self._world_of(G) is None and self.accum_u is None and fused_x and joint
+                    and not (G.pair_i or G.pair_b) and G.A0 is None and G.B0 is None)
+
+    def _gen_front_merged(self, G):
+        th = self.theta.data
+        M = (self.method, self.H, self.K, self.m)
+        lone = bool(getattr(G, 'skip_v', False))
+        e0 = self._mark()
+        if not lone:
+            self._launch_test_net_here(G)
+        with self._side(1, e0):
+            fwd = [self._job(G, 'i'), self._job(G, 'b')]
+            self._ode_fwd_multi(fwd, G.t, th, *M, zero16=self.scal, narrow=self._narrow_ok(fwd, alone=False, forward=True),
+                             prio_drop=self.prio_drop['G'])
+            self._reaction(G)
+            sweep_x = [self._job(G, 'i', want_x=True)]
+            self._ode_bwd_multi(sweep_x, G.t, th, *M, want_x=True, want_params=False,
+                             narrow=self._narrow_ok(sweep_x, alone=False, params=False))
+            e_x = self._mark()
+        self._join(e_x)
+        self._contract(G, self.adam_u, with_bdry=True)
+        res_M = dict(u=G.u, ref=G.v, coef=G.Vol / G.Nglob / G.L * G.s3_scale, base=G.Vol / G.Nglob,
+                     weak=dict(w=G.w, c=G.c, cp=G.cp, ckappa=G.ck),
+                     merged=dict(ref=G.h, coef=2.0 * self.alpha / G.Nglob, base=self.pollution, scal=self.scal))
+        res_b = dict(u=G.ub, ref=G.g, coef=2.0 * self.alpha / (G.Nbglob * G.Lb), base=0.0, first_only=False)
+        sweeps = [dict(self._job(G, 'i', None, G.slabA[:G.ns_u]), res=res_M),
+                  dict(self._job(G, 'b', None, G.slabA[G.ns_u:]), res=res_b)]
+        self._ode_bwd_multi(sweeps, G.t, th, *M, want_x=False, want_params=True, narrow=self._narrow_ok(sweeps, alone=False))
+        G.sumA_ready = False
+
     def begin_substep(self, which, accumulate):
         name, P = ('accum_u', self.Pu) if which == 'u' else ('accum_v', self.Pv)
         if which == 'u':
@@ -1040,7 +1076,9 @@
                 KN.pair_fold(self.scal, G.Vol, G.Nglob)
             KN.losses(self.scal, G.L, G.Lb, G.Vol, G.Nglob, G.Nbglob, self.alpha, step=st['step'], init_off=G.init_off,
                       bdry_off=G.bdry_off)
-        if world is None and getattr(G, 'sumA_ready', False) and acc is None:
+        if world is None and getattr(G, 'merged', False):
+            KN.adam(self.theta.data, G.slabA, st['m'], st['v'], st['step'], lr, gsum_out=self.grad_u, bump_step=-1, **lag)
+        elif world is None and getattr(G, 'sumA_ready', False) and acc is None:
             KN.adam(self.theta.data, None, st['m'], st['v'], st['step'], lr, gslabB=G.slabB, scal=self.scal,
                     gextraA=G.sumA, gsum_out=self.grad_u, bump_step=-1, **lag)
         elif world is None:
diff --git a/xnode_wan_pde_solver_amd/kernels.py b/xnode_wan_pde_solver_amd/kernels.py
--- a/xnode_wan_pde_solver_amd/kernels.py
+++ b/xnode_wan_pde_solver_amd/kernels.py
@@ -214,6 +214,11 @@
             a.res_first_only, a.res_u, a.res_ref = 2, _p(res['u']), _p(res['ref'])
             a.res_w_per_point, a.res_w, a.res_c, a.res_cp = int(wpp), _p(wk['w']), _p(wk.get('c')), _p(wk.get('cp'))
             a.res_kappa2 = 2.0 * float(wk.get('ckappa', 0.0))
+            mg = res.get('merged')
+            if mg is not None:
+                _chk(mg.get('ref'), F64, (N,), 'res.merged.ref'); _chk(mg.get('scal'), F64, None, 'res.merged.scal')
+                a.res_first_only, a.res_scal, a.res_refA = 3, _p(mg.get('scal')), _p(mg.get('ref'))
+                a.res_coefA, a.res_baseA = float(mg['coef']), float(mg['base'])
         else:
             first = bool(res['first_only'])
             _chk(res['u'], F64, (L, N), 'res.u'); _chk(res['ref'], F64, (N,) if first else (L, N), 'res.ref')
diff --git a/xnode_wan_pde_solver_amd/options.py b/xnode_wan_pde_solver_amd/options.py
--- a/xnode_wan_pde_solver_amd/options.py
+++ b/xnode_wan_pde_solver_amd/options.py
@@ -29,6 +29,7 @@
     narrow_tiles: Optional[str] = None
     narrow_tiles_alone: str = '256:256:64'
     early_slab_sum: bool = True
+    merged_sweep: bool = True
     compact_tiles: int = 320
     prio_drop_A: Optional[int] = None
     prio_drop_X: int = 0
@@ -70,6 +71,7 @@
         o.narrow_tiles = os.environ.get('XW_NARROW_TILES') or None
         o.narrow_tiles_alone = os.environ.get('XW_NARROW_TILES_ALONE') or o.narrow_tiles_alone
         o.early_slab_sum = _flag('XW_EARLY_SLAB_SUM', o.early_slab_sum)
+        o.merged_sweep = _flag('XW_MERGED_SWEEP', o.merged_sweep)
         o.compact_tiles = _int('XW_COMPACT_TILES', o.compact_tiles)
         o.prio_drop_A = _int('XW_PRIO_DROP_A', None)
         o.prio_drop_X = _int('XW_PRIO_DROP_X', o.prio_drop_X)
```

Result: faster. 2173, median of 6 (+2.2%).
